# cp2k/dbcsr

Hardware: AMD Instinct MI355X
Metric: block-sparse multiply GFLOP/s (fp64) (higher is better)
Workload: dtype f64; 1 GPU; config2_32768_23x23_fill10_fp64; M=32768, c_nblks=2030625, nproducts=29207882, k_passes=1, parallelism=1 GPU

## Files before the change

### dbcsr_amd/csrc/mm_engine.hip

```cpp
#include <hip/hip_runtime.h>

#include <cstdio>
#include <cstdlib>
#include <cstring>
#include <algorithm>
#include <new>
#include <vector>

#include "../../include/dbcsr_amd_mm.h"
#include "common.h"
#include "smm_core.h"
#include "mm_types.h"
#include "mm_jit.h"

#include "mm_workspace.h"
#include "mm_symbolic.h"
#include "mm_numeric_f64.h"
#include "mm_numeric_f64_big.h"
#include "mm_numeric_f64_small.h"
#include "mm_mid.h"
#include "mm_numeric_f32.h"
#include "mm_aux.h"
#ifdef DBCSR_AMD_EXPERIMENTS
#include "mm_lab_api.h"
#include "mm_group.h"
#include "mm_group64.h"
#include "mm_dma.h"
#include "mm_tile_index.h"
#include "mm_band_index.h"
#endif
namespace dbcsr_amd {

#include "mm_engine_state.h"
#include "mm_engine_env.h"
#include "mm_engine_launch.h"
#include "mm_engine_plan.h"
#ifdef DBCSR_AMD_EXPERIMENTS
#include "mm_engine_lab.h"
#endif


static int build_product_lists(Engine* E, bool reuse, const dbcsr_amd_bcsr* a, const dbcsr_amd_bcsr* b, const dbcsr_amd_bcsr* c_in, dbcsr_amd_bcsr* c_out,
                               hipStream_t st) {
  const int nbr = E->facts.nbr, W = E->W, nbc = b->nblkcols, nJ = (nbc + 63) / 64;
  const int64_t nblk = E->facts.c_nblks;
  const uint32_t* cin_bm = E->have_cin ? E->cin_bm.p : nullptr;
  const int* cin_pre = E->have_cin ? E->cin_pre.p : nullptr;
  if (reuse) {
    ACC_CHECK(hipMemcpyAsync(c_out->col_i, E->plan_c_col_i.p, sizeof(int32_t) * (size_t)nblk, hipMemcpyDeviceToDevice, st));
    ACC_CHECK(hipMemcpyAsync(c_out->blk_p, E->plan_c_blk_p.p, sizeof(int64_t) * (size_t)nblk, hipMemcpyDeviceToDevice, st));
  } else if (E->rows_kernels) {
    if (E->tmp_i32.ensure((size_t)nblk + 1)) return -1;
    ACC_CHECK(hipMemsetAsync(E->tmp_i32.p, 0, sizeof(int) * (size_t)nblk, st));
    hipLaunchKernelGGL(fill_products_rows, grid_for((int64_t)nbr * 64), dim3(256), 0, st, a->row_p, a->col_i, a->blk_p, a->col_blk_size, b->row_p,
                       b->col_i, b->blk_p, E->c_bm.p, E->c_pre.p, c_out->row_p, E->prod_start.p, nbr, W, E->tmp_i32.p, E->entries.p, E->filter);
    hipLaunchKernelGGL(finish_descs_grid, grid_for((int64_t)nbr * nJ * 64), dim3(256), 0, st, c_in->row_p, c_in->blk_p, c_out->row_blk_size,
                       c_out->col_blk_size, cin_bm, cin_pre, E->c_bm.p, E->c_pre.p, c_out->row_p, E->c_blk_p_ws.p, E->prod_start.p,
                       E->prod_cnt.p, nbr, W, nJ, c_out->col_i, c_out->blk_p, E->descs.p);
  } else if (E->grid_kernels) {
    hipLaunchKernelGGL(fill_products_grid, grid_for((int64_t)nbr * nJ * 64), dim3(256), 0, st, a->row_p, a->col_i, a->blk_p, b->row_p,
                       b->blk_p, c_in->row_p, c_in->blk_p, a->row_blk_size, a->col_blk_size, b->col_blk_size, E->b_bm.p, E->b_pre.p,
                       cin_bm, cin_pre, E->c_bm.p, E->c_pre.p, c_out->row_p, E->prod_start.p, E->c_blk_p_ws.p, nbr, nbc, W, nJ, c_out->col_i,
                       c_out->blk_p, E->descs.p, E->entries.p, E->filter);
  } else {
    hipLaunchKernelGGL(fill_products, grid_for((int64_t)nbr * W), dim3(256), 0, st, a->row_p, a->col_i, a->blk_p, b->row_p, b->blk_p,
                       c_in->row_p, c_in->blk_p, a->row_blk_size, a->col_blk_size, b->col_blk_size, E->b_bm.p, E->b_pre.p,
                       cin_bm, cin_pre, E->c_bm.p, E->c_pre.p, c_out->row_p, E->prod_start.p, E->c_blk_p_ws.p, nbr, W, c_out->col_i, c_out->blk_p,
                       E->descs.p, E->entries.p);
  }
  return 0;
}

template <typename T>
static NumericArgs<T> numeric_args(Engine* E, hipStream_t st, const dbcsr_amd_bcsr* a, const dbcsr_amd_bcsr* b, const dbcsr_amd_bcsr* c_in,
                                   const dbcsr_amd_bcsr* c_out, double alpha, double beta, const Work* work, double* norms, bool reuse) {
  return NumericArgs<T>{st, E->descs.p, E->facts.c_nblks, E->entries.p, static_cast<const T*>(a->data), static_cast<const T*>(b->data),
                        static_cast<T*>(c_out->data), static_cast<const T*>(c_in->data), (T)alpha, (T)beta, E->facts.skip_empty, E->order.p, work, norms,
                        a, b, c_out, reuse};
}

static int launch_classes_f64(Engine* E, const NumericArgs<double>& p, const NumericChoice& c) {
  const SizeFacts& F = E->facts;
  int njit = 0, ngen = 0, nmid = 0, jit_mask = 0, nlaunch = 0;
  const int nside = E->lab.class_streams > 1 ? E->lab.class_streams - 1 : 0;
  if (nside) {
    if (!E->fork_ev) ACC_CHECK(hipEventCreateWithFlags(&E->fork_ev, hipEventDisableTiming));
    ACC_CHECK(hipEventRecord(E->fork_ev, p.st));
    for (int i = 0; i < nside; ++i) {
      if (!E->side_stream[i]) {
        ACC_CHECK(hipStreamCreateWithFlags(&E->side_stream[i], hipStreamNonBlocking));
        ACC_CHECK(hipEventCreateWithFlags(&E->join_ev[i], hipEventDisableTiming));
      }
      ACC_CHECK(hipStreamWaitEvent(E->side_stream[i], E->fork_ev, 0));
    }
  }
  for (int k = 0; k < kNumClasses; ++k) {
    if (E->cls_len[k] == 0) continue;
    NumericArgs<double> q = p.segment(E->cls_off[k]);
    const int slot = nlaunch++ % (nside + 1);
    if (slot) q.st = E->side_stream[slot - 1];
    const unsigned npos = (unsigned)(8 * E->cls_len[k]);
    const int cm = k < 9 ? F.cls_m[k / 3] : 0, cn = k < 9 ? F.cls_n[k % 3] : 0;
    ClassKernel ck;
    if (k < 9 && c.mid_class_mode && mid_f64_serves(cm, cn, c.mid_class_mode)) {
      if (!launch_mid_f64(q, (cm + 3) / 4, (cn + 3) / 4, false, npos, (std::max(cm, cn) + 3) / 4)) return -1;
      ++nmid;
      jit_mask |= 1 << k;
    } else if (k < 9 && cm > 0 && cn > 0 && jit_class_kernel(cm, cn, F.cls_k[0], F.cls_k[1], F.cls_k[2], E->lab.class_g, &ck) == 0) {
      long nblk_l = (long)q.nblk;
      void* args[] = {&q.descs, &nblk_l, &q.entries, &q.a, &q.b, &q.c_out, &q.c_in, &q.alpha, &q.beta, &q.skip_empty, &q.order, &q.work, &q.norms};
      const unsigned cw = E->lab.class_g == 1 ? (unsigned)c.ww : 4u;
      ACC_CHECK(hipModuleLaunchKernel(ck.fn, npos / cw / (unsigned)E->lab.class_g, 1, 1, 64 * cw, 1, 1, (unsigned)(cw * ck.wave_lds), q.st, args, nullptr));
      ++njit;
      jit_mask |= 1 << k;
    } else {
      launch_lds_f64(q, c, (unsigned)(8 * E->cls_len[k] / 4) * 4u / (unsigned)c.ww);
      ++ngen;
    }
  }
  for (int i = 0; i < nside; ++i) {
    ACC_CHECK(hipEventRecord(E->join_ev[i], E->side_stream[i]));
    ACC_CHECK(hipStreamWaitEvent(p.st, E->join_ev[i], 0));
  }
  if (p.norms) {
    ClassSet cs;
    for (int r = 0; r < 3; ++r) cs.m[r] = F.cls_m[r], cs.n[r] = F.cls_n[r];
    cs.jit_mask = jit_mask;
    hipLaunchKernelGGL(block_norms_unserved_classes, grid_for(p.nblk * 64), dim3(256), 0, p.st, p.descs, p.nblk, p.c_out, cs, p.norms);
  }
  char slab[24] = "";
  if (nmid > 0) snprintf(slab, sizeof slab, "%d slab + ", nmid);
  snprintf(E->last_kernel, sizeof E->last_kernel, "%s%d jit + %s%d generic launches; m {%d,%d,%d} n {%d,%d,%d} k {%d,%d,%d}]", c.name, njit, slab, ngen,
           F.cls_m[0], F.cls_m[1], F.cls_m[2], F.cls_n[0], F.cls_n[1], F.cls_n[2], F.cls_k[0], F.cls_k[1], F.cls_k[2]);
  return 0;
}

static int launch_f64(Engine* E, const NumericChoice& c, const NumericArgs<double>& p, const LabSwitches& lab) {
  const SizeFacts& F = E->facts;
  const int64_t npos = 8 * F.order_len;
  snprintf(E->last_kernel, sizeof E->last_kernel, "%s", c.name);
  if (p.norms && c.leaves_norms) E->norms_data = p.c_out, E->norms_nblks = p.nblk;
  switch (c.family) {
    case Family::f64_tiny:
      if (c.grid > 0) launch_tiny_f64(p, c, F.max_k <= 4);
      return 0;
    case Family::f64_small8:
      if (c.grid > 0) launch_small_f64(p, c, npos);
      return 0;
    case Family::f64_mid:
      return launch_mid_f64(p, c.mid_rb, c.mid_cb, F.min_m != F.max_m || F.min_n != F.max_n, c.grid, (std::max(F.max_m, F.max_n) + 3) / 4) ? 0 : -1;
    case Family::f64_classes: return launch_classes_f64(E, p, c);
    case Family::f64_hot: return launch_hot_f64(p, c, F.hot_m, F.hot_n, F.hot_k, c.flags, c.variant) ? 0 : -1;
    case Family::f64_pipe: launch_pipe_f64(p, c, npos); return 0;
    case Family::f64_lds: launch_lds_f64(p, c, c.grid); return 0;
    case Family::f64_big: return launch_big_f64(p, c, big_tiles(F.max_m), big_tiles(F.max_n)) ? 0 : -1;
    case Family::f64_generic:
      hipLaunchKernelGGL(mm_numeric_f64, dim3(c.grid), dim3(256), 0, p.st, p.descs, p.nblk, p.entries, p.a, p.b, p.c_out, p.c_in, p.alpha, p.beta, c.flags);
      return 0;
#ifdef DBCSR_AMD_EXPERIMENTS
    case Family::f64_group: case Family::f64_tile: case Family::f64_band: case Family::f64_dma: case Family::f64_persistent: return launch_lab_f64(E, c, p, lab);
#endif
    default: return -1;
  }
}

static int launch_f32(Engine* E, const NumericChoice& c, const NumericArgs<float>& p) {
  const SizeFacts& F = E->facts;
  snprintf(E->last_kernel, sizeof E->last_kernel, "%s", c.name);
  switch (c.family) {
    case Family::f32_classes:
      for (int k = 0; k < kNumClasses; ++k)
        if (E->cls_len[k] != 0) launch_lds_f32(p.segment(E->cls_off[k]), c, (unsigned)(8 * E->cls_len[k] / c.ww));
      return 0;
    case Family::f32_direct: return launch_hot_f32_direct(p, c, F.hot_m, F.hot_n, F.hot_k, c.flags, c.slim) ? 0 : -1;
    case Family::f32_hot: return launch_hot_f32(p, c, F.hot_m, F.hot_n, F.hot_k) ? 0 : -1;
    case Family::f32_lds: launch_lds_f32(p, c, c.grid); return 0;
    case Family::f32_generic:
      hipLaunchKernelGGL(mm_numeric_f32, dim3(c.grid), dim3(256), 0, p.st, p.descs, p.nblk, p.entries, p.a, p.b, p.c_out, p.c_in, p.alpha, p.beta, c.flags);
      return 0;
#ifdef DBCSR_AMD_EXPERIMENTS
    case Family::f32_group: {
      const int rc = run_group_f32(E, p, c.group_R);
      if (rc == 0 && F.other_sizes()) launch_hot_f32_direct(p, c, F.hot_m, F.hot_n, F.hot_k, c.flags | 2, false);
      if (rc != 1) return rc;
      LabSwitches lab = E->lab;
      lab.f32_group = 0;
      return launch_f32(E, choose_numeric(F, E->sw, lab), p);
    }
#endif
    default: return -1;
  }
}

}

using namespace dbcsr_amd;

extern "C" {

int dbcsr_amd_mm_create(void** handle) {
  if (!handle) return -1;
  Engine* E = new (std::nothrow) Engine();
  if (!E) return -1;
  hipError_t e = hipHostMalloc(reinterpret_cast<void**>(&E->host_scalars), 16 * sizeof(int64_t), hipHostMallocDefault);
  if (e != hipSuccess) {
    delete E;
    return check(e, "hipHostMalloc", __FILE__, __LINE__);
  }
  if (hipHostMalloc(reinterpret_cast<void**>(&E->cls_host_hist), 3 * 33 * sizeof(int), hipHostMallocDefault) != hipSuccess ||
      hipHostMalloc(reinterpret_cast<void**>(&E->cls_host_lens), (2 * kNumClasses + 1) * sizeof(int64_t), hipHostMallocDefault) != hipSuccess)
    return -1;
  if (hipHostMalloc(reinterpret_cast<void**>(&E->plan_host_flag), sizeof(int), hipHostMallocDefault) != hipSuccess) return -1;
  engine_read_env(E);
  for (int i = 0; i < 3; ++i) {
    e = hipEventCreate(&E->ev[i]);
    if (e != hipSuccess) return check(e, "hipEventCreate", __FILE__, __LINE__);
  }
  *handle = E;
  return 0;
}

int dbcsr_amd_mm_timing(void* handle, float* ms_fill, float* ms_numeric) {
  Engine* E = static_cast<Engine*>(handle);
  if (!E || !E->timed) return -1;
  ACC_CHECK(hipEventSynchronize(E->ev[2]));
  float f = 0.f, n = 0.f;
  ACC_CHECK(hipEventElapsedTime(&f, E->ev[0], E->ev[1]));
  ACC_CHECK(hipEventElapsedTime(&n, E->ev[1], E->ev[2]));
  if (ms_fill) *ms_fill = f;
  if (ms_numeric) *ms_numeric = n;
  return 0;
}

int dbcsr_amd_mm_destroy(void* handle) {
  if (!handle) return 0;
  Engine* E = static_cast<Engine*>(handle);
  if (E->host_scalars) (void)hipHostFree(E->host_scalars);
  if (E->plan_host_flag) (void)hipHostFree(E->plan_host_flag);
  if (E->cls_host_hist) (void)hipHostFree(E->cls_host_hist);
  if (E->cls_host_lens) (void)hipHostFree(E->cls_host_lens);
  for (int i = 0; i < 3; ++i)
    if (E->ev[i]) (void)hipEventDestroy(E->ev[i]);
  for (int i = 0; i < 3; ++i) {
    if (E->side_stream[i]) (void)hipStreamDestroy(E->side_stream[i]);
    if (E->join_ev[i]) (void)hipEventDestroy(E->join_ev[i]);
  }
  if (E->fork_ev) (void)hipEventDestroy(E->fork_ev);
  delete E;
  return 0;
}

int dbcsr_amd_mm_symbolic(void* handle, const dbcsr_amd_bcsr* a, const dbcsr_amd_bcsr* b, const dbcsr_amd_bcsr* c_in,
                          int retain_sparsity, int32_t* c_out_row_p, dbcsr_amd_mm_counts* counts, void* stream) {
  return dbcsr_amd_mm_symbolic_filtered(handle, dbcsr_type_real_8, 1.0, 0.0, a, b, c_in, retain_sparsity, c_out_row_p, counts, stream);
}

int dbcsr_amd_mm_symbolic_filtered(void* handle, libsmm_acc_data_t datatype, double alpha, double filter_eps, const dbcsr_amd_bcsr* a,
                                   const dbcsr_amd_bcsr* b, const dbcsr_amd_bcsr* c_in, int retain_sparsity, int32_t* c_out_row_p,
                                   dbcsr_amd_mm_counts* counts, void* stream) {
  Engine* E = static_cast<Engine*>(handle);
  if (!E || !a || !b || !c_in || !c_out_row_p || !counts) return -1;
  E->drop_pending = 0.0;
  const bool filtering = filter_eps > 0.0;
  if (filtering && datatype != dbcsr_type_real_8 && datatype != dbcsr_type_real_4) return -10;
  if (a->nblkcols != b->nblkrows || a->nblkrows != c_in->nblkrows || b->nblkcols != c_in->nblkcols) {
    fprintf(stderr, "dbcsr_amd_mm_symbolic: incompatible block dimensions\n");
    return -2;
  }
  hipStream_t st = stream_of(stream);
  const int nbr = a->nblkrows, nbk = a->nblkcols, nbc = b->nblkcols;
  const int W = (nbc + 31) / 32;
  if (!filtering) {
    const int hit = plan_matches(E, a, b, c_in, retain_sparsity ? 1 : 0, st);
    if (hit < 0) return -1;
    if (hit) {
      long long off = 0;
      const void* ptr[12];
      long long n[12];
      plan_segments(a, b, c_in, ptr, n);
      for (int i = 0; i < 12; ++i) off += n[i];
      ACC_CHECK(hipMemcpyAsync(c_out_row_p, E->plan_words.p + off, sizeof(int32_t) * ((size_t)nbr + 1), hipMemcpyDeviceToDevice, st));
      *counts = E->plan_counts;
      E->norms_data = nullptr;
      E->filter = FilterArgs{nullptr, nullptr, 0.0f};
      E->valid = true;
      E->plan_hit = true;
      ++E->plan_hits;
      return 0;
    }
  }
  plan_invalidate(E);
  E->valid = false;
  E->facts.nbr = nbr;
  E->facts.nbc = nbc;
  E->W = W;
  E->facts.retain = retain_sparsity != 0;
  E->norms_data = nullptr;
  E->have_cin = c_in->nblks > 0;
  if (E->b_bm.ensure((size_t)nbk * W + 1) || E->b_pre.ensure((size_t)nbk * W + 1) || E->c_bm.ensure((size_t)nbr * W + 1) ||
      E->c_pre.ensure((size_t)nbr * W + 1) || E->row_nnz.ensure((size_t)nbr + 1) || E->dev_scalars.ensure(16))
    return -1;
  if (E->have_cin && (E->cin_bm.ensure((size_t)nbr * W + 1) || E->cin_pre.ensure((size_t)nbr * W + 1))) return -1;
  ACC_CHECK(hipMemsetAsync(E->dev_scalars.p, 0, 16 * sizeof(unsigned long long), st));
  {
    static const int init[6] = {0, -0x7fffffff, 0, -0x7fffffff, 0, -0x7fffffff};
    ACC_CHECK(hipMemcpyAsync(E->dev_scalars.p + 4, init, sizeof(init), hipMemcpyHostToDevice, st));
  }
  if (nbr == 0 || nbc == 0) {
    ACC_CHECK(hipMemsetAsync(c_out_row_p, 0, sizeof(int32_t) * ((size_t)nbr + 1), st));
    ACC_CHECK(hipStreamSynchronize(st));
    counts->c_nblks = counts->c_nze = counts->nproducts = counts->flop = 0;
    E->facts.c_nblks = 0;
    E->facts.nproducts = 0;
    E->valid = true;
    return 0;
  }
  ACC_CHECK(hipMemsetAsync(E->b_bm.p, 0, sizeof(uint32_t) * (size_t)nbk * W, st));
  if (nbk > 0) {
    hipLaunchKernelGGL(bitmap_from_index, grid_for((int64_t)nbk * 64), dim3(256), 0, st, b->row_p, b->col_i, nbk, W, E->b_bm.p);
    hipLaunchKernelGGL(row_prefix, grid_for((int64_t)nbk * 64), dim3(256), 0, st, E->b_bm.p, nbk, W, E->b_pre.p, (int*)nullptr);
  }
  if (E->have_cin) {
    ACC_CHECK(hipMemsetAsync(E->cin_bm.p, 0, sizeof(uint32_t) * (size_t)nbr * W, st));
    hipLaunchKernelGGL(bitmap_from_index, grid_for((int64_t)nbr * 64), dim3(256), 0, st, c_in->row_p, c_in->col_i, nbr, W,
                       E->cin_bm.p);
    hipLaunchKernelGGL(row_prefix, grid_for((int64_t)nbr * 64), dim3(256), 0, st, E->cin_bm.p, nbr, W, E->cin_pre.p, (int*)nullptr);
  }
  E->filter = FilterArgs{nullptr, nullptr, 0.0f};
  if (filtering) {
    if (E->a_norms.ensure((size_t)a->nblks + 1) || E->b_norms.ensure((size_t)b->nblks + 1)) return -1;
    const int sa = row_split(nbr, a->nblks), sb = row_split(nbk, b->nblks);
    if (datatype == dbcsr_type_real_8) {
      hipLaunchKernelGGL((bcsr_block_norms<double>), grid_for((int64_t)nbr * sa * 64), dim3(256), 0, st, a->row_p, a->col_i, a->blk_p,
                         static_cast<const double*>(a->data), a->row_blk_size, a->col_blk_size, nbr, sa, 1.0, E->a_norms.p, (double*)nullptr);
      hipLaunchKernelGGL((bcsr_block_norms<double>), grid_for((int64_t)nbk * sb * 64), dim3(256), 0, st, b->row_p, b->col_i, b->blk_p,
                         static_cast<const double*>(b->data), b->row_blk_size, b->col_blk_size, nbk, sb, alpha, E->b_norms.p, (double*)nullptr);
    } else {
      hipLaunchKernelGGL((bcsr_block_norms<float>), grid_for((int64_t)nbr * sa * 64), dim3(256), 0, st, a->row_p, a->col_i, a->blk_p,
                         static_cast<const float*>(a->data), a->row_blk_size, a->col_blk_size, nbr, sa, 1.0, E->a_norms.p, (double*)nullptr);
      hipLaunchKernelGGL((bcsr_block_norms<float>), grid_for((int64_t)nbk * sb * 64), dim3(256), 0, st, b->row_p, b->col_i, b->blk_p,
                         static_cast<const float*>(b->data), b->row_blk_size, b->col_blk_size, nbk, sb, alpha, E->b_norms.p, (double*)nullptr);
    }
    E->filter = FilterArgs{E->a_norms.p, E->b_norms.p, (float)filter_eps};
  }
  const double prod_est = (double)a->nblks * ((double)b->nblks / (double)std::max(nbk, 1));
  const bool sparse_guess = E->force_symbolic == 3 || (E->force_symbolic == 0 && nbr >= 2048 && prod_est < 0.6 * (double)nbr * (double)nbc);
  if (filtering && sparse_guess && !retain_sparsity) {
    if (E->have_cin)
      ACC_CHECK(hipMemcpyAsync(E->c_bm.p, E->cin_bm.p, sizeof(uint32_t) * (size_t)nbr * W, hipMemcpyDeviceToDevice, st));
    else
      ACC_CHECK(hipMemsetAsync(E->c_bm.p, 0, sizeof(uint32_t) * (size_t)nbr * W, st));
    hipLaunchKernelGGL(c_bitmap_rows_filtered, grid_for((int64_t)nbr * 64), dim3(256), 0, st, a->row_p, a->col_i, b->row_p, b->col_i, nbr, W,
                       E->facts.canonical_c, E->filter, E->c_bm.p);
  } else if (filtering)
    hipLaunchKernelGGL(c_bitmap_filtered, grid_for((int64_t)nbr * ((nbc + 63) / 64) * 64), dim3(256), 0, st, a->row_p, a->col_i, b->row_p,
                       E->b_bm.p, E->b_pre.p, E->have_cin ? E->cin_bm.p : (const uint32_t*)nullptr, nbr, nbc, W, (nbc + 63) / 64,
                       retain_sparsity ? 1 : 0, E->facts.canonical_c, E->filter, E->c_bm.p);
  else
    hipLaunchKernelGGL(c_bitmap, grid_for((int64_t)nbr * W), dim3(256), 0, st, a->row_p, a->col_i, E->b_bm.p,
                       E->have_cin ? E->cin_bm.p : (const uint32_t*)nullptr, nbr, W, retain_sparsity ? 1 : 0, E->facts.canonical_c, E->c_bm.p);
  hipLaunchKernelGGL(row_prefix, grid_for((int64_t)nbr * 64), dim3(256), 0, st, E->c_bm.p, nbr, W, E->c_pre.p, E->row_nnz.p);
  int64_t* dsc = reinterpret_cast<int64_t*>(E->dev_scalars.p);
  if (exclusive_scan<int32_t>(E, E->row_nnz.p, nbr, c_out_row_p, dsc + 0, true, st)) return -1;
  if (E->sw.use_classes > 0 && E->cls_hist.ensure(3 * 33)) return -1;
  hipLaunchKernelGGL(block_size_stats, dim3(3), dim3(256), 0, st, a->row_blk_size, nbr, a->col_blk_size, nbk, b->col_blk_size, nbc,
                     reinterpret_cast<int*>(E->dev_scalars.p + 4), reinterpret_cast<int*>(E->dev_scalars.p + 8), reinterpret_cast<int*>(E->dev_scalars.p + 11),
                     E->sw.use_classes > 0 ? E->cls_hist.p : (int*)nullptr);
  if (E->sw.use_classes > 0) ACC_CHECK(hipMemcpyAsync(E->cls_host_hist, E->cls_hist.p, 3 * 33 * sizeof(int), hipMemcpyDeviceToHost, st));
  ACC_CHECK(hipMemcpyAsync(E->host_scalars, dsc, 13 * sizeof(int64_t), hipMemcpyDeviceToHost, st));
  ACC_CHECK(hipStreamSynchronize(st));
  const int64_t c_nblks = E->host_scalars[0];
  {
    const int* mx = reinterpret_cast<const int*>(E->host_scalars + 4);
    E->facts.max_m = mx[0]; E->facts.min_m = -mx[1];
    E->facts.max_k = mx[2]; E->facts.min_k = -mx[3];
    E->facts.max_n = mx[4]; E->facts.min_n = -mx[5];
    if (E->facts.max_k > 0xffff || E->facts.max_m > 0x7fff || E->facts.max_n > 0x7fff) {
      fprintf(stderr, "dbcsr_amd_mm_symbolic: block sizes above 32767 (m, n) / 65535 (k) are not supported (packed 16-bit extents)\n");
      return -1;
    }
    const int* md = reinterpret_cast<const int*>(E->host_scalars + 8);
    const bool dominant = 10ll * md[1] >= 9ll * nbr && 10ll * md[3] >= 9ll * nbk && 10ll * md[5] >= 9ll * nbc;
    E->facts.hot_m = dominant ? md[0] : 0;
    E->facts.hot_k = dominant ? md[2] : 0;
    E->facts.hot_n = dominant ? md[4] : 0;
    E->facts.hot_cnt_m = md[1], E->facts.hot_cnt_k = md[3], E->facts.hot_cnt_n = md[5];
    const int* um = reinterpret_cast<const int*>(E->host_scalars + 11);
    E->facts.units_m = um[0], E->facts.units_cnt_m = um[1], E->facts.units_n = um[2], E->facts.units_cnt_n = um[3];
  }
  E->facts.c_nblks = c_nblks;
  choose_classes(&E->facts, E->sw, E->cls_host_hist);
  double mean_k = E->facts.max_k, mean_n = E->facts.max_n;
  if (E->sw.use_classes > 0 && E->facts.max_k <= 32 && E->facts.max_n <= 32 && E->facts.min_k >= 1 && E->facts.min_n >= 1) {
    double sk = 0, ck = 0, sn = 0, cn = 0;
    for (int sz = 1; sz <= 32; ++sz) {
      sn += (double)sz * E->cls_host_hist[33 + sz];
      cn += E->cls_host_hist[33 + sz];
      sk += (double)sz * E->cls_host_hist[66 + sz];
      ck += E->cls_host_hist[66 + sz];
    }
    if (ck > 0 && cn > 0) mean_k = sk / ck, mean_n = sn / cn;
  }
  const int64_t b_bytes_est = (int64_t)((double)b->nblks * mean_k * mean_n * (double)sizeof(double));
  int NP = (int)std::min<int64_t>((b_bytes_est + E->panel_bytes - 1) / E->panel_bytes, (int64_t)W);
  if (NP < 1) NP = 1;
  const int PW = (W + NP - 1) / NP;
  NP = (W + PW - 1) / PW;
  const int R = (nbr + 7) / 8;
  int RG = E->lab.row_group > 0 ? E->lab.row_group : 1;
  RG = std::max(1, std::min(RG, R));
  const int NG = (R + RG - 1) / RG;
  const int nkeys = (E->facts.cls_mode ? kNumClasses : 1) * 8 * NP * (E->facts.cls_mode ? R : NG);
  if (E->order_cnt.ensure((size_t)nkeys + 1) || E->order_base.ensure((size_t)nkeys + 1)) return -1;
  if (E->facts.cls_mode) {
    if (E->cls_row.ensure((size_t)nbr + 1) || E->cls_col.ensure((size_t)nbc + 1) || E->cls_col_bm.ensure((size_t)4 * W + 1) ||
        E->cls_lens.ensure(2 * kNumClasses + 1) || E->cls_vpos.ensure((size_t)nbr + 1) || E->cls_vrow.ensure((size_t)nbr + 1))
      return -1;
    hipLaunchKernelGGL(class_ids, grid_for(nbr), dim3(256), 0, st, a->row_blk_size, nbr, E->facts.cls_m[0], E->facts.cls_m[1], E->facts.cls_m[2], E->cls_row.p);
    hipLaunchKernelGGL(class_ids, grid_for(nbc), dim3(256), 0, st, b->col_blk_size, nbc, E->facts.cls_n[0], E->facts.cls_n[1], E->facts.cls_n[2], E->cls_col.p);
    hipLaunchKernelGGL(class_col_bitmaps, grid_for(W), dim3(256), 0, st, E->cls_col.p, nbc, W, E->cls_col_bm.p);
    hipLaunchKernelGGL(class_row_deal, dim3(1), dim3(256), 0, st, E->cls_row.p, nbr, E->cls_vpos.p, E->cls_vrow.p);
    hipLaunchKernelGGL(order_count_cls, grid_for(nkeys), dim3(256), 0, st, E->c_bm.p, E->cls_row.p, E->cls_col_bm.p, E->cls_vrow.p, nbr, W, PW, NP, R,
                       E->order_cnt.p);
    if (exclusive_scan<int64_t>(E, E->order_cnt.p, nkeys, E->order_base.p, nullptr, false, st)) return -1;
    hipLaunchKernelGGL(order_len_cls, dim3(1), dim3(1), 0, st, E->order_base.p, c_nblks, NP, R, E->cls_lens.p);
    ACC_CHECK(hipMemcpyAsync(E->cls_host_lens, E->cls_lens.p, (2 * kNumClasses + 1) * sizeof(int64_t), hipMemcpyDeviceToHost, st));
  } else {
  hipLaunchKernelGGL(order_count, grid_for(nkeys), dim3(256), 0, st, E->c_pre.p, E->row_nnz.p, nbr, W, PW, NP, NG, RG, E->order_cnt.p);
  if (exclusive_scan<int64_t>(E, E->order_cnt.p, nkeys, E->order_base.p, nullptr, false, st)) return -1;
  hipLaunchKernelGGL(order_len, dim3(1), dim3(1), 0, st, E->order_base.p, c_nblks, NP, NG, dsc + 7);
  }
  if (E->prod_cnt.ensure((size_t)c_nblks + 1) || E->blk_nze.ensure((size_t)c_nblks + 1) || E->prod_start.ensure((size_t)c_nblks + 1) ||
      E->c_blk_p_ws.ensure((size_t)c_nblks + 1))
    return -1;
  const int nJ = (nbc + 63) / 64;
  E->grid_kernels = filtering || (((int64_t)nbr * nJ * 64 <= 256 * std::max<int64_t>(c_nblks, 1)) && !E->force_word_kernels);
  E->rows_kernels = E->force_symbolic == 3 || (E->force_symbolic == 0 && nbr >= 2048 && 10 * c_nblks < 6 * (int64_t)nbr * nbc);
  if (E->rows_kernels) {
    E->grid_kernels = false;
    ACC_CHECK(hipMemsetAsync(E->prod_cnt.p, 0, sizeof(int) * (size_t)c_nblks, st));
    hipLaunchKernelGGL(block_sizes_rows, grid_for((int64_t)nbr * W), dim3(256), 0, st, E->c_bm.p, E->c_pre.p, c_out_row_p, a->row_blk_size,
                       b->col_blk_size, nbr, W, E->blk_nze.p);
    hipLaunchKernelGGL(count_products_rows, grid_for((int64_t)nbr * 64), dim3(256), 0, st, a->row_p, a->col_i, a->row_blk_size, a->col_blk_size,
                       b->col_blk_size, b->row_p, b->col_i, E->c_bm.p, E->c_pre.p, c_out_row_p, nbr, W, E->prod_cnt.p, E->dev_scalars.p + 3,
                       E->filter);
  } else if (E->grid_kernels)
    hipLaunchKernelGGL(count_products_grid, grid_for((int64_t)nbr * nJ * 64), dim3(256), 0, st, a->row_p, a->col_i, a->row_blk_size,
                       a->col_blk_size, b->col_blk_size, E->b_bm.p, E->c_bm.p, E->c_pre.p, c_out_row_p, nbr, nbc, W, nJ,
                       E->prod_cnt.p, E->blk_nze.p, E->dev_scalars.p + 3, b->row_p, E->b_pre.p, E->filter);
  else
    hipLaunchKernelGGL(count_products, grid_for((int64_t)nbr * W), dim3(256), 0, st, a->row_p, a->col_i, a->row_blk_size,
                       a->col_blk_size, b->col_blk_size, E->b_bm.p, E->c_bm.p, E->c_pre.p, c_out_row_p, nbr, W, E->prod_cnt.p,
                       E->blk_nze.p, E->dev_scalars.p + 3);
  if (exclusive_scan<int64_t>(E, E->prod_cnt.p, c_nblks, E->prod_start.p, dsc + 2, false, st)) return -1;
  if (exclusive_scan<int64_t>(E, E->blk_nze.p, c_nblks, E->c_blk_p_ws.p, dsc + 1, false, st)) return -1;
  ACC_CHECK(hipMemcpyAsync(E->host_scalars, dsc, 8 * sizeof(int64_t), hipMemcpyDeviceToHost, st));
  ACC_CHECK(hipStreamSynchronize(st));
  E->facts.order_len = E->host_scalars[7];
  if (E->facts.cls_mode) {
    for (int c = 0; c < kNumClasses; ++c) {
      E->cls_len[c] = E->cls_host_lens[c];
      E->cls_off[c] = E->cls_host_lens[kNumClasses + c];
    }
    const int64_t total = E->cls_host_lens[2 * kNumClasses];
    E->facts.order_len = total / 8;
    if (E->order.ensure((size_t)total + 64)) return -1;
    if (total > 0) {
      ACC_CHECK(hipMemsetAsync(E->order.p, 0xff, sizeof(int) * ((size_t)total + 64), st));
      hipLaunchKernelGGL(order_fill_cls, grid_for((int64_t)nbr * W), dim3(256), 0, st, E->c_bm.p, E->c_pre.p, c_out_row_p, E->cls_row.p,
                         E->cls_col_bm.p, E->order_base.p, E->cls_lens.p, E->cls_vpos.p, nbr, W, PW, NP, R, E->order.p);
    }
  } else {
  if (E->order.ensure((size_t)(8 * E->facts.order_len) + 64)) return -1;
  if (E->facts.order_len > 0) {
    ACC_CHECK(hipMemsetAsync(E->order.p, 0xff, sizeof(int) * ((size_t)(8 * E->facts.order_len) + 64), st));
    hipLaunchKernelGGL(order_fill, grid_for((int64_t)nbr * W), dim3(256), 0, st, E->c_bm.p, E->c_pre.p, E->row_nnz.p, c_out_row_p,
                       E->order_base.p, nbr, W, PW, NP, NG, RG, E->facts.order_len, E->order.p);
  }
  }
  counts->c_nblks = E->host_scalars[0];
  counts->c_nze = E->host_scalars[1];
  counts->nproducts = E->host_scalars[2];
  counts->flop = E->host_scalars[3];
  E->facts.c_nblks = counts->c_nblks;
  E->facts.nproducts = counts->nproducts;
  E->valid = true;
  ++E->plan_misses;
  if (!filtering) {
    if (plan_save(E, a, b, c_in, retain_sparsity ? 1 : 0, c_out_row_p, *counts, st)) return -1;
  } else {
    plan_invalidate(E);
  }
  return check(hipGetLastError(), "dbcsr_amd_mm_symbolic", __FILE__, __LINE__);
}

int dbcsr_amd_mm_numeric(void* handle, libsmm_acc_data_t datatype, double alpha, const dbcsr_amd_bcsr* a, const dbcsr_amd_bcsr* b,
                         double beta, const dbcsr_amd_bcsr* c_in, dbcsr_amd_bcsr* c_out, void* stream) {
  Engine* E = static_cast<Engine*>(handle);
  if (!E || !E->valid || !a || !b || !c_in || !c_out) {
    fprintf(stderr, "dbcsr_amd_mm_numeric: no valid symbolic phase for this handle\n");
    return -1;
  }
  if (datatype != dbcsr_type_real_8 && datatype != dbcsr_type_real_4) return -10;
  hipStream_t st = stream_of(stream);
  SizeFacts& F = E->facts;
  const int64_t nblk = F.c_nblks;
  if (nblk == 0) return 0;
  const bool reuse = E->plan_hit && E->plan_numeric;
  if (!reuse) {
    E->work_built = false;
#ifdef DBCSR_AMD_EXPERIMENTS
    E->ls.forget_plan();
#endif
  }
  if (E->entries.ensure((size_t)F.nproducts + 1) || E->descs.ensure((size_t)nblk + 1)) return -1;
  ACC_CHECK(hipEventRecord(E->ev[0], st));
  if (int rc = build_product_lists(E, reuse, a, b, c_in, c_out, st)) return rc;
  F.nbc = b->nblkcols;
  F.fp64 = datatype == dbcsr_type_real_8;
  F.filter_active = E->filter.a_norms != nullptr;
  F.skip_empty = (c_out->data == c_in->data && F.retain && beta == 1.0) ? 1 : 0;
  const NumericChoice ch = choose_numeric(F, E->sw, E->lab);
  const Work* work = nullptr;
  if (ch.work) {
    const int64_t npos = 8 * F.order_len;
    if (!(reuse && E->work_built)) {
      if (E->work.ensure((size_t)npos + 1)) return -1;
      hipLaunchKernelGGL(build_work, grid_for(npos), dim3(256), 0, st, E->order.p, npos, E->descs.p, nblk, E->entries.p, E->work.p);
      E->work_built = true;
    }
    work = E->work.p;
  }
  double* norms = nullptr;
  E->norms_data = nullptr;
  if (ch.norms) {
    if (E->norms64.ensure((size_t)nblk + 1)) return -1;
    norms = E->norms64.p;
  }
  const double drop = norms ? E->drop_pending : 0.0;
  E->drop_pending = 0.0;
  E->unwritten_below = 0.0;
  if (norms) {
    hipLaunchKernelGGL(store_scalar_f64, dim3(1), dim3(1), 0, st, norms + nblk, drop);
    E->unwritten_below = drop;
  }
  ACC_CHECK(hipEventRecord(E->ev[1], st));
  if ((F.fp64 ? launch_f64(E, ch, numeric_args<double>(E, st, a, b, c_in, c_out, alpha, beta, work, norms, reuse), E->lab)
              : launch_f32(E, ch, numeric_args<float>(E, st, a, b, c_in, c_out, alpha, beta, work, norms, reuse))) != 0) {
    fprintf(stderr, "dbcsr_amd_mm_numeric: launching %s failed\n", E->last_kernel);
    return -1;
  }
  ACC_CHECK(hipEventRecord(E->ev[2], st));
  E->timed = true;
  c_out->nblks = nblk;
  if (E->plan_saved && !E->plan_numeric) {
    if (E->plan_c_col_i.ensure((size_t)nblk + 1) || E->plan_c_blk_p.ensure((size_t)nblk + 1)) return -1;
    ACC_CHECK(hipMemcpyAsync(E->plan_c_col_i.p, c_out->col_i, sizeof(int32_t) * (size_t)nblk, hipMemcpyDeviceToDevice, st));
    ACC_CHECK(hipMemcpyAsync(E->plan_c_blk_p.p, c_out->blk_p, sizeof(int64_t) * (size_t)nblk, hipMemcpyDeviceToDevice, st));
    E->plan_numeric = true;
  }
  return check(hipGetLastError(), "dbcsr_amd_mm_numeric", __FILE__, __LINE__);
}

#include "mm_engine_ops.h"

}
```

### dbcsr_amd/csrc/mm_engine_ops.h

```cpp
#ifndef DBCSR_AMD_MM_ENGINE_OPS_H
#define DBCSR_AMD_MM_ENGINE_OPS_H

int dbcsr_amd_mm_init_c(void* handle, libsmm_acc_data_t datatype, double beta, const dbcsr_amd_bcsr* c_in, dbcsr_amd_bcsr* c_out,
                        void* stream) {
  Engine* E = static_cast<Engine*>(handle);
  if (E) E->plan_numeric = false;
  if (!E || !E->valid || !c_in || !c_out) {
    fprintf(stderr, "dbcsr_amd_mm_init_c: no valid symbolic phase for this handle\n");
    return -1;
  }
  if (datatype != dbcsr_type_real_8 && datatype != dbcsr_type_real_4) return -10;
  hipStream_t st = stream_of(stream);
  const int nbr = E->facts.nbr, W = E->W;
  const int64_t nblk = E->facts.c_nblks;
  c_out->nblks = nblk;
  if (nblk == 0) return 0;
  if (E->descs.ensure((size_t)nblk + 1)) return -1;
  hipLaunchKernelGGL(emit_index, grid_for((int64_t)nbr * W), dim3(256), 0, st, c_in->row_p, c_in->blk_p, c_out->row_blk_size,
                     c_out->col_blk_size, E->have_cin ? E->cin_bm.p : (const uint32_t*)nullptr,
                     E->have_cin ? E->cin_pre.p : (const int*)nullptr, E->c_bm.p, E->c_pre.p, c_out->row_p, E->c_blk_p_ws.p, nbr, W,
                     c_out->col_i, c_out->blk_p, E->descs.p);
  if (datatype == dbcsr_type_real_8)
    hipLaunchKernelGGL((init_c_blocks<double>), grid_for(nblk * 64), dim3(256), 0, st, E->descs.p, nblk,
                       static_cast<double*>(c_out->data), static_cast<const double*>(c_in->data), beta);
  else
    hipLaunchKernelGGL((init_c_blocks<float>), grid_for(nblk * 64), dim3(256), 0, st, E->descs.p, nblk,
                       static_cast<float*>(c_out->data), static_cast<const float*>(c_in->data), (float)beta);
  return check(hipGetLastError(), "dbcsr_amd_mm_init_c", __FILE__, __LINE__);
}


static int element_offsets(Engine* E, const int* sizes, int n, DevBuf<int64_t>& off, hipStream_t st) {
  if (off.ensure((size_t)n + 1)) return -1;
  return exclusive_scan<int64_t>(E, sizes, n, off.p, nullptr, false, st);
}

static Window make_window(const dbcsr_amd_bcsr* m, int64_t row_lo, int64_t row_hi, int64_t col_lo, int64_t col_hi) {
  (void)m;
  const int64_t big = 0x7fffffff;
  Window w;
  w.r0 = (int)(row_lo < 0 ? 0 : row_lo);
  w.r1 = (int)(row_hi < 0 || row_hi > big ? big : row_hi);
  w.c0 = (int)(col_lo < 0 ? 0 : col_lo);
  w.c1 = (int)(col_hi < 0 || col_hi > big ? big : col_hi);
  return w;
}

int dbcsr_amd_bcsr_crop_count(void* handle, libsmm_acc_data_t datatype, const dbcsr_amd_bcsr* m, int64_t row_lo, int64_t row_hi,
                              int64_t col_lo, int64_t col_hi, int32_t* new_row_p, int64_t* new_nblks, int64_t* new_nze, void* stream) {
  Engine* E = static_cast<Engine*>(handle);
  if (E) plan_invalidate(E);
  if (!E || !m || !new_row_p || !new_nblks || !new_nze) return -1;
  if (datatype != dbcsr_type_real_8 && datatype != dbcsr_type_real_4) return -10;
  hipStream_t st = stream_of(stream);
  const int nbr = m->nblkrows;
  const int64_t nb = m->nblks;
  E->valid = false;
  E->flt_nblks = nb;
  E->flt_new_nblks = -1;
  E->crop_win = make_window(m, row_lo, row_hi, col_lo, col_hi);
  E->crop_pending = true;
  if (E->keep.ensure((size_t)nb + 1) || E->blk_nze.ensure((size_t)nb + 1) || E->row_nnz.ensure((size_t)nbr + 1) ||
      E->prod_start.ensure((size_t)nb + 1) || E->c_blk_p_ws.ensure((size_t)nb + 1) || E->dev_scalars.ensure(16))
    return -1;
  int64_t* dsc = reinterpret_cast<int64_t*>(E->dev_scalars.p);
  ACC_CHECK(hipMemsetAsync(dsc, 0, 16 * sizeof(int64_t), st));
  if (element_offsets(E, m->row_blk_size, nbr, E->off_a, st)) return -1;
  if (element_offsets(E, m->col_blk_size, m->nblkcols, E->off_b, st)) return -1;
  if (nbr > 0 && nb > 0)
    hipLaunchKernelGGL(crop_flags, grid_for((int64_t)nbr * 64), dim3(256), 0, st, m->row_p, m->col_i, m->row_blk_size, m->col_blk_size,
                       E->off_a.p, E->off_b.p, nbr, E->crop_win, E->keep.p, E->blk_nze.p, E->row_nnz.p);
  else if (nbr > 0)
    ACC_CHECK(hipMemsetAsync(E->row_nnz.p, 0, sizeof(int) * (size_t)nbr, st));
  if (exclusive_scan<int32_t>(E, E->row_nnz.p, nbr, new_row_p, dsc + 0, true, st)) return -1;
  if (exclusive_scan<int64_t>(E, E->keep.p, nb, E->prod_start.p, nullptr, false, st)) return -1;
  if (exclusive_scan<int64_t>(E, E->blk_nze.p, nb, E->c_blk_p_ws.p, dsc + 1, false, st)) return -1;
  ACC_CHECK(hipMemcpyAsync(E->host_scalars, dsc, 2 * sizeof(int64_t), hipMemcpyDeviceToHost, st));
  ACC_CHECK(hipStreamSynchronize(st));
  *new_nblks = E->host_scalars[0];
  *new_nze = E->host_scalars[1];
  return check(hipGetLastError(), "dbcsr_amd_bcsr_crop_count", __FILE__, __LINE__);
}

int dbcsr_amd_bcsr_crop_apply(void* handle, libsmm_acc_data_t datatype, const dbcsr_amd_bcsr* src, dbcsr_amd_bcsr* dst, void* stream) {
  Engine* E = static_cast<Engine*>(handle);
  if (E) plan_invalidate(E);
  if (!E || !src || !dst || !E->crop_pending || E->flt_nblks != src->nblks) return -1;
  E->crop_pending = false;
  hipStream_t st = stream_of(stream);
  const int nbr = src->nblkrows;
  if (nbr == 0 || src->nblks == 0) return 0;
  if (datatype == dbcsr_type_real_8)
    hipLaunchKernelGGL((crop_compact<double>), grid_for((int64_t)nbr * 64), dim3(256), 0, st, src->row_p, src->col_i, src->blk_p,
                       static_cast<const double*>(src->data), src->row_blk_size, src->col_blk_size, E->off_a.p, E->off_b.p, nbr,
                       E->crop_win, E->keep.p, E->prod_start.p, E->c_blk_p_ws.p, dst->col_i, dst->blk_p, static_cast<double*>(dst->data));
  else if (datatype == dbcsr_type_real_4)
    hipLaunchKernelGGL((crop_compact<float>), grid_for((int64_t)nbr * 64), dim3(256), 0, st, src->row_p, src->col_i, src->blk_p,
                       static_cast<const float*>(src->data), src->row_blk_size, src->col_blk_size, E->off_a.p, E->off_b.p, nbr,
                       E->crop_win, E->keep.p, E->prod_start.p, E->c_blk_p_ws.p, dst->col_i, dst->blk_p, static_cast<float*>(dst->data));
  else
    return -10;
  return check(hipGetLastError(), "dbcsr_amd_bcsr_crop_apply", __FILE__, __LINE__);
}

int dbcsr_amd_bcsr_scale_window(void* handle, libsmm_acc_data_t datatype, dbcsr_amd_bcsr* m, double beta, int64_t row_lo, int64_t row_hi,
                                int64_t col_lo, int64_t col_hi, void* stream) {
  Engine* E = static_cast<Engine*>(handle);
  if (!E || !m) return -1;
  hipStream_t st = stream_of(stream);
  const int nbr = m->nblkrows;
  if (nbr == 0 || m->nblks == 0) return 0;
  const Window w = make_window(m, row_lo, row_hi, col_lo, col_hi);
  if (element_offsets(E, m->row_blk_size, nbr, E->off_a, st)) return -1;
  if (element_offsets(E, m->col_blk_size, m->nblkcols, E->off_b, st)) return -1;
  if (datatype == dbcsr_type_real_8)
    hipLaunchKernelGGL((scale_window<double>), grid_for((int64_t)nbr * 64), dim3(256), 0, st, m->row_p, m->col_i, m->blk_p,
                       static_cast<double*>(m->data), m->row_blk_size, m->col_blk_size, E->off_a.p, E->off_b.p, nbr, w, beta);
  else if (datatype == dbcsr_type_real_4)
    hipLaunchKernelGGL((scale_window<float>), grid_for((int64_t)nbr * 64), dim3(256), 0, st, m->row_p, m->col_i, m->blk_p,
                       static_cast<float*>(m->data), m->row_blk_size, m->col_blk_size, E->off_a.p, E->off_b.p, nbr, w, (float)beta);
  else
    return -10;
  return check(hipGetLastError(), "dbcsr_amd_bcsr_scale_window", __FILE__, __LINE__);
}

int dbcsr_amd_bcsr_filter_count(void* handle, libsmm_acc_data_t datatype, const dbcsr_amd_bcsr* m, double eps, int32_t* new_row_p,
                                int64_t* new_nblks, int64_t* new_nze, void* stream) {
  Engine* E = static_cast<Engine*>(handle);
  if (E) plan_invalidate(E);
  if (!E || !m || !new_row_p || !new_nblks || !new_nze) return -1;
  if (datatype != dbcsr_type_real_8 && datatype != dbcsr_type_real_4) return -10;
  hipStream_t st = stream_of(stream);
  const int nbr = m->nblkrows;
  const int64_t nb = m->nblks;
  E->valid = false;
  E->flt_nblks = nb;
  E->flt_new_nblks = -1;
  if (E->norms64.ensure((size_t)nb + 1) || E->keep.ensure((size_t)nb + 1) || E->blk_nze.ensure((size_t)nb + 1) ||
      E->row_nnz.ensure((size_t)nbr + 1) || E->prod_start.ensure((size_t)nb + 1) || E->c_blk_p_ws.ensure((size_t)nb + 1) ||
      E->dev_scalars.ensure(16))
    return -1;
  int64_t* dsc = reinterpret_cast<int64_t*>(E->dev_scalars.p);
  ACC_CHECK(hipMemsetAsync(dsc, 0, 16 * sizeof(int64_t), st));
  const bool have_norms = E->norms_data != nullptr && E->norms_data == m->data && E->norms_nblks == nb && datatype == dbcsr_type_real_8;
  if (have_norms && E->unwritten_below > eps * eps) {
    fprintf(stderr, "dbcsr_amd_bcsr_filter_count: this matrix was multiplied with a final filter of eps^2 = %g announced (dbcsr_amd_mm_expect_filter); "
                    "blocks below that were not written and cannot be kept with eps^2 = %g\n", E->unwritten_below, eps * eps);
    return -3;
  }
  E->norms_data = nullptr;
  E->unwritten_below = 0.0;
  if (nbr > 0 && nb > 0) {
    const int sm = row_split(nbr, nb);
    if (have_norms) {
    } else if (datatype == dbcsr_type_real_8)
      hipLaunchKernelGGL((bcsr_block_norms<double>), grid_for((int64_t)nbr * sm * 64), dim3(256), 0, st, m->row_p, m->col_i, m->blk_p,
                         static_cast<const double*>(m->data), m->row_blk_size, m->col_blk_size, nbr, sm, 1.0, (float*)nullptr, E->norms64.p);
    else
      hipLaunchKernelGGL((bcsr_block_norms<float>), grid_for((int64_t)nbr * sm * 64), dim3(256), 0, st, m->row_p, m->col_i, m->blk_p,
                         static_cast<const float*>(m->data), m->row_blk_size, m->col_blk_size, nbr, sm, 1.0, (float*)nullptr, E->norms64.p);
    hipLaunchKernelGGL(filter_flags, grid_for((int64_t)nbr * 64), dim3(256), 0, st, E->norms64.p, nb, m->row_p, m->col_i, m->row_blk_size,
                       m->col_blk_size, nbr, eps * eps, E->keep.p, E->blk_nze.p, E->row_nnz.p);
  }
  if (exclusive_scan<int32_t>(E, E->row_nnz.p, nbr, new_row_p, dsc + 0, true, st)) return -1;
  if (exclusive_scan<int64_t>(E, E->keep.p, nb, E->prod_start.p, nullptr, false, st)) return -1;
  if (exclusive_scan<int64_t>(E, E->blk_nze.p, nb, E->c_blk_p_ws.p, dsc + 1, false, st)) return -1;
  ACC_CHECK(hipMemcpyAsync(E->host_scalars, dsc, 2 * sizeof(int64_t), hipMemcpyDeviceToHost, st));
  ACC_CHECK(hipStreamSynchronize(st));
  *new_nblks = E->host_scalars[0];
  *new_nze = E->host_scalars[1];
  E->flt_new_nblks = E->host_scalars[0];
  return check(hipGetLastError(), "dbcsr_amd_bcsr_filter_count", __FILE__, __LINE__);
}

int dbcsr_amd_bcsr_filter_apply(void* handle, libsmm_acc_data_t datatype, const dbcsr_amd_bcsr* src, dbcsr_amd_bcsr* dst, void* stream) {
  Engine* E = static_cast<Engine*>(handle);
  if (E) plan_invalidate(E);
  if (!E || !src || !dst || E->flt_nblks != src->nblks) return -1;
  hipStream_t st = stream_of(stream);
  const int nbr = src->nblkrows;
  if (nbr == 0 || src->nblks == 0) return 0;
  const int sc = row_split(nbr, src->nblks);
  if (datatype == dbcsr_type_real_8)
    hipLaunchKernelGGL((filter_compact<double>), grid_for((int64_t)nbr * sc * 64), dim3(256), 0, st, src->row_p, src->col_i, src->blk_p,
                       static_cast<const double*>(src->data), src->row_blk_size, src->col_blk_size, nbr, sc, E->keep.p, E->prod_start.p,
                       E->c_blk_p_ws.p, dst->col_i, dst->blk_p, static_cast<double*>(dst->data));
  else if (datatype == dbcsr_type_real_4)
    hipLaunchKernelGGL((filter_compact<float>), grid_for((int64_t)nbr * sc * 64), dim3(256), 0, st, src->row_p, src->col_i, src->blk_p,
                       static_cast<const float*>(src->data), src->row_blk_size, src->col_blk_size, nbr, sc, E->keep.p, E->prod_start.p,
                       E->c_blk_p_ws.p, dst->col_i, dst->blk_p, static_cast<float*>(dst->data));
  else
    return -10;
  return check(hipGetLastError(), "dbcsr_amd_bcsr_filter_apply", __FILE__, __LINE__);
}

int dbcsr_amd_bcsr_filter_apply_index(void* handle, const dbcsr_amd_bcsr* src, dbcsr_amd_bcsr* dst, void* stream) {
  Engine* E = static_cast<Engine*>(handle);
  if (E) plan_invalidate(E);
  if (!E || !src || !dst || E->flt_new_nblks < 0 || E->flt_nblks != src->nblks || dst->data != src->data) return -1;
  hipStream_t st = stream_of(stream);
  if (src->nblkrows == 0 || src->nblks == 0 || E->flt_new_nblks == 0) return 0;
  if (!dst->col_i || !dst->blk_p) return -1;
  hipLaunchKernelGGL(filter_compact_index, grid_for(src->nblks), dim3(256), 0, st, src->col_i, src->blk_p, (int64_t)src->nblks, E->keep.p,
                     E->prod_start.p, E->flt_new_nblks, dst->col_i, dst->blk_p);
  return check(hipGetLastError(), "dbcsr_amd_bcsr_filter_apply_index", __FILE__, __LINE__);
}

int dbcsr_amd_mm_set_filter_in_place(void* handle, int on) {
  Engine* E = static_cast<Engine*>(handle);
  if (!E) return -1;
  E->filter_in_place = on ? 1 : 0;
  return 0;
}

int dbcsr_amd_bcsr_checksum(void* handle, libsmm_acc_data_t datatype, const dbcsr_amd_bcsr* m, double* out2, void* stream) {
  Engine* E = static_cast<Engine*>(handle);
  if (!E || !m || !out2) return -1;
  hipStream_t st = stream_of(stream);
  const int nbr = m->nblkrows;
  out2[0] = out2[1] = 0.0;
  if (nbr == 0 || m->nblks == 0) return 0;
  if (E->row_sums.ensure((size_t)2 * nbr + 2)) return -1;
  if (element_offsets(E, m->row_blk_size, nbr, E->off_a, st)) return -1;
  if (element_offsets(E, m->col_blk_size, m->nblkcols, E->off_b, st)) return -1;
  if (datatype == dbcsr_type_real_8)
    hipLaunchKernelGGL((checksum_blocks<double>), grid_for((int64_t)nbr * 64), dim3(256), 0, st, m->row_p, m->col_i, m->blk_p,
                       static_cast<const double*>(m->data), m->row_blk_size, m->col_blk_size, E->off_a.p, E->off_b.p, nbr,
                       E->row_sums.p);
  else if (datatype == dbcsr_type_real_4)
    hipLaunchKernelGGL((checksum_blocks<float>), grid_for((int64_t)nbr * 64), dim3(256), 0, st, m->row_p, m->col_i, m->blk_p,
                       static_cast<const float*>(m->data), m->row_blk_size, m->col_blk_size, E->off_a.p, E->off_b.p, nbr,
                       E->row_sums.p);
  else
    return -10;
  hipLaunchKernelGGL(checksum_final, dim3(1), dim3(256), 0, st, E->row_sums.p, nbr, E->row_sums.p + 2 * (size_t)nbr);
  ACC_CHECK(hipMemcpyAsync(E->host_scalars + 4, E->row_sums.p + 2 * (size_t)nbr, 2 * sizeof(double), hipMemcpyDeviceToHost, st));
  ACC_CHECK(hipStreamSynchronize(st));
  memcpy(out2, E->host_scalars + 4, 2 * sizeof(double));
  return 0;
}

int dbcsr_amd_bcsr_fill_random(void* handle, libsmm_acc_data_t datatype, const dbcsr_amd_bcsr* m, int counter, void* stream) {
  return dbcsr_amd_bcsr_fill_random_dist(handle, datatype, m, counter, nullptr, nullptr, m ? m->nblkrows : 0, stream);
}

int dbcsr_amd_bcsr_fill_random_dist(void* handle, libsmm_acc_data_t datatype, const dbcsr_amd_bcsr* m, int counter,
                                    const int32_t* row_gid, const int32_t* col_gid, int32_t nblkrows_global, void* stream) {
  if (!handle || !m) return -1;
  hipStream_t st = stream_of(stream);
  if (m->nblks == 0) return 0;
  if (datatype == dbcsr_type_real_8)
    hipLaunchKernelGGL(fill_random_f64, grid_for((int64_t)m->nblkrows * 64), dim3(256), 0, st, m->row_p, m->col_i, m->blk_p,
                       static_cast<double*>(m->data), m->row_blk_size, m->col_blk_size, m->nblkrows, m->nblkcols, counter, row_gid, col_gid,
                       nblkrows_global);
  else if (datatype == dbcsr_type_real_4)
    hipLaunchKernelGGL(fill_random_f32, grid_for(m->nblks), dim3(256), 0, st, m->row_p, m->col_i, m->blk_p,
                       static_cast<float*>(m->data), m->row_blk_size, m->col_blk_size, m->nblkrows, m->nblkcols, counter, row_gid, col_gid,
                       nblkrows_global);
  else
    return -10;
  return check(hipGetLastError(), "dbcsr_amd_bcsr_fill_random", __FILE__, __LINE__);
}

int dbcsr_amd_bcsr_transpose(void* handle, libsmm_acc_data_t datatype, const dbcsr_amd_bcsr* src, dbcsr_amd_bcsr* dst, void* stream) {
  Engine* E = static_cast<Engine*>(handle);
  if (E) plan_invalidate(E);
  if (!E || !src || !dst) return -1;
  if (datatype != dbcsr_type_real_8 && datatype != dbcsr_type_real_4) return -10;
  hipStream_t st = stream_of(stream);
  const int s_nbr = src->nblkrows, t_nbr = src->nblkcols;
  const int Wt = (s_nbr + 31) / 32;
  E->valid = false;
  if (E->c_bm.ensure((size_t)t_nbr * Wt + 1) || E->c_pre.ensure((size_t)t_nbr * Wt + 1) || E->row_nnz.ensure((size_t)t_nbr + 1) ||
      E->blk_nze.ensure((size_t)src->nblks + 1) || E->c_blk_p_ws.ensure((size_t)src->nblks + 1))
    return -1;
  if (t_nbr == 0) return 0;
  ACC_CHECK(hipMemsetAsync(E->c_bm.p, 0, sizeof(uint32_t) * (size_t)t_nbr * Wt, st));
  if (s_nbr > 0) hipLaunchKernelGGL(transpose_mark, grid_for((int64_t)s_nbr * 64), dim3(256), 0, st, src->row_p, src->col_i, s_nbr, Wt, E->c_bm.p);
  hipLaunchKernelGGL(row_prefix, grid_for((int64_t)t_nbr * 64), dim3(256), 0, st, E->c_bm.p, t_nbr, Wt, E->c_pre.p, E->row_nnz.p);
  if (exclusive_scan<int32_t>(E, E->row_nnz.p, t_nbr, dst->row_p, nullptr, true, st)) return -1;
  if (src->nblks > 0) {
    hipLaunchKernelGGL(transpose_sizes, grid_for((int64_t)t_nbr * Wt), dim3(256), 0, st, E->c_bm.p, E->c_pre.p, dst->row_p,
                       src->row_blk_size, src->col_blk_size, t_nbr, Wt, E->blk_nze.p);
    if (exclusive_scan<int64_t>(E, E->blk_nze.p, src->nblks, E->c_blk_p_ws.p, nullptr, false, st)) return -1;
    if (datatype == dbcsr_type_real_8)
      hipLaunchKernelGGL((transpose_fill<double>), grid_for((int64_t)s_nbr * 64), dim3(256), 0, st, src->row_p, src->col_i, src->blk_p,
                         static_cast<const double*>(src->data), src->row_blk_size, src->col_blk_size, E->c_bm.p, E->c_pre.p, dst->row_p,
                         E->c_blk_p_ws.p, s_nbr, Wt, dst->col_i, dst->blk_p, static_cast<double*>(dst->data));
    else
      hipLaunchKernelGGL((transpose_fill<float>), grid_for((int64_t)s_nbr * 64), dim3(256), 0, st, src->row_p, src->col_i, src->blk_p,
                         static_cast<const float*>(src->data), src->row_blk_size, src->col_blk_size, E->c_bm.p, E->c_pre.p, dst->row_p,
                         E->c_blk_p_ws.p, s_nbr, Wt, dst->col_i, dst->blk_p, static_cast<float*>(dst->data));
  }
  dst->nblks = src->nblks;
  return check(hipGetLastError(), "dbcsr_amd_bcsr_transpose", __FILE__, __LINE__);
}

int dbcsr_amd_bcsr_desymmetrize_count(void* handle, const dbcsr_amd_bcsr* src, int32_t* dst_row_p, int64_t* nblks, int64_t* nze, void* stream) {
  return dbcsr_amd_bcsr_twin_count(handle, src, 0, dst_row_p, nblks, nze, stream);
}

int dbcsr_amd_bcsr_desymmetrize_apply(void* handle, libsmm_acc_data_t datatype, const dbcsr_amd_bcsr* src, int antisymmetric, dbcsr_amd_bcsr* dst,
                                      void* stream) {
  return dbcsr_amd_bcsr_twin_apply(handle, datatype, src, 0, antisymmetric, dst, stream);
}

int dbcsr_amd_mm_set_canonical_product(void* handle, int on) {
  Engine* E = static_cast<Engine*>(handle);
  if (E) plan_invalidate(E);
  if (!E) return -1;
  E->facts.canonical_c = on ? 1 : 0;
  return 0;
}

int dbcsr_amd_bcsr_twin_count(void* handle, const dbcsr_amd_bcsr* src, int mode, int32_t* dst_row_p, int64_t* nblks, int64_t* nze, void* stream) {
  Engine* E = static_cast<Engine*>(handle);
  if (E) plan_invalidate(E);
  if (!E || !src || !dst_row_p || !nblks || !nze || src->nblkrows != src->nblkcols || mode < 0 || mode > 2) return -1;
  hipStream_t st = stream_of(stream);
  const int nbr = src->nblkrows, W = (nbr + 31) / 32;
  E->valid = false;
  *nblks = *nze = 0;
  if (nbr == 0) return 0;
  if (E->c_bm.ensure((size_t)nbr * W + 1) || E->c_pre.ensure((size_t)nbr * W + 1) || E->row_nnz.ensure((size_t)nbr + 1) ||
      E->blk_nze.ensure(2 * (size_t)src->nblks + 1) || E->c_blk_p_ws.ensure(2 * (size_t)src->nblks + 1) || E->dev_scalars.ensure(16))
    return -1;
  int64_t* dsc = reinterpret_cast<int64_t*>(E->dev_scalars.p);
  ACC_CHECK(hipMemsetAsync(E->c_bm.p, 0, sizeof(uint32_t) * (size_t)nbr * W, st));
  hipLaunchKernelGGL(desym_mark, grid_for((int64_t)nbr * 64), dim3(256), 0, st, src->row_p, src->col_i, nbr, W, mode, E->c_bm.p);
  hipLaunchKernelGGL(row_prefix, grid_for((int64_t)nbr * 64), dim3(256), 0, st, E->c_bm.p, nbr, W, E->c_pre.p, E->row_nnz.p);
  if (exclusive_scan<int32_t>(E, E->row_nnz.p, nbr, dst_row_p, dsc + 0, true, st)) return -1;
  hipLaunchKernelGGL(transpose_sizes, grid_for((int64_t)nbr * W), dim3(256), 0, st, E->c_bm.p, E->c_pre.p, dst_row_p, src->row_blk_size,
                     src->col_blk_size, nbr, W, E->blk_nze.p);
  ACC_CHECK(hipMemcpyAsync(E->host_scalars, dsc, sizeof(int64_t), hipMemcpyDeviceToHost, st));
  ACC_CHECK(hipStreamSynchronize(st));
  *nblks = E->host_scalars[0];
  if (exclusive_scan<int64_t>(E, E->blk_nze.p, *nblks, E->c_blk_p_ws.p, dsc + 1, false, st)) return -1;
  ACC_CHECK(hipMemcpyAsync(E->host_scalars, dsc, 2 * sizeof(int64_t), hipMemcpyDeviceToHost, st));
  ACC_CHECK(hipStreamSynchronize(st));
  *nze = E->host_scalars[1];
  return check(hipGetLastError(), "dbcsr_amd_bcsr_twin_count", __FILE__, __LINE__);
}

int dbcsr_amd_bcsr_twin_apply(void* handle, libsmm_acc_data_t datatype, const dbcsr_amd_bcsr* src, int mode, int antisymmetric, dbcsr_amd_bcsr* dst,
                              void* stream) {
  Engine* E = static_cast<Engine*>(handle);
  if (E) plan_invalidate(E);
  if (!E || !src || !dst || src->nblkrows != src->nblkcols || mode < 0 || mode > 2) return -1;
  if (datatype != dbcsr_type_real_8 && datatype != dbcsr_type_real_4) return -10;
  hipStream_t st = stream_of(stream);
  const int nbr = src->nblkrows, W = (nbr + 31) / 32;
  if (nbr == 0 || src->nblks == 0) return 0;
  if (datatype == dbcsr_type_real_8)
    hipLaunchKernelGGL((desym_fill<double>), grid_for((int64_t)nbr * 64), dim3(256), 0, st, src->row_p, src->col_i, src->blk_p,
                       static_cast<const double*>(src->data), src->row_blk_size, E->c_bm.p, E->c_pre.p, dst->row_p, E->c_blk_p_ws.p, nbr, W,
                       antisymmetric ? -1.0 : 1.0, mode, dst->col_i, dst->blk_p, static_cast<double*>(dst->data));
  else
    hipLaunchKernelGGL((desym_fill<float>), grid_for((int64_t)nbr * 64), dim3(256), 0, st, src->row_p, src->col_i, src->blk_p,
                       static_cast<const float*>(src->data), src->row_blk_size, E->c_bm.p, E->c_pre.p, dst->row_p, E->c_blk_p_ws.p, nbr, W,
                       antisymmetric ? -1.0f : 1.0f, mode, dst->col_i, dst->blk_p, static_cast<float*>(dst->data));
  return check(hipGetLastError(), "dbcsr_amd_bcsr_twin_apply", __FILE__, __LINE__);
}

int dbcsr_amd_mm_stats(void* handle, dbcsr_amd_mnk_stat* out, int max_entries, int* n_entries, void* stream) {
  Engine* E = static_cast<Engine*>(handle);
  if (!E || !n_entries || (max_entries > 0 && !out)) return -1;
  *n_entries = 0;
  if (!E->valid || !E->timed || E->facts.c_nblks == 0) return 0;
  hipStream_t st = stream_of(stream);
  if (E->stat_table.ensure(2 * (size_t)kStatSlots + 2)) return -1;
  unsigned long long* keys = E->stat_table.p;
  unsigned long long* counts = keys + kStatSlots;
  int* overflow = reinterpret_cast<int*>(counts + kStatSlots);
  ACC_CHECK(hipMemsetAsync(keys, 0, sizeof(unsigned long long) * (2 * (size_t)kStatSlots + 2), st));
  hipLaunchKernelGGL(mnk_histogram, grid_for(E->facts.c_nblks), dim3(256), 0, st, E->descs.p, E->facts.c_nblks, E->entries.p, keys, counts, overflow);
  std::vector<unsigned long long> host(2 * (size_t)kStatSlots + 2);
  ACC_CHECK(hipMemcpyAsync(host.data(), keys, sizeof(unsigned long long) * host.size(), hipMemcpyDeviceToHost, st));
  ACC_CHECK(hipStreamSynchronize(st));
  if (*reinterpret_cast<const int*>(&host[2 * (size_t)kStatSlots])) {
    fprintf(stderr, "dbcsr_amd_mm_stats: more than %d distinct (m, n, k) triples\n", kStatSlots);
    return -1;
  }
  std::vector<dbcsr_amd_mnk_stat> all;
  for (int i = 0; i < kStatSlots; ++i)
    if (host[i]) {
      dbcsr_amd_mnk_stat r;
      r.m = (int32_t)(host[i] & 0xffffu);
      r.n = (int32_t)((host[i] >> 16) & 0xffffu);
      r.k = (int32_t)((host[i] >> 32) & 0x7fffffffu);
      r.reserved = 0;
      r.nproducts = (int64_t)host[kStatSlots + i];
      r.flop = 2ll * r.m * r.n * r.k * r.nproducts;
      all.push_back(r);
    }
  std::sort(all.begin(), all.end(), [](const dbcsr_amd_mnk_stat& a, const dbcsr_amd_mnk_stat& b) {
    return a.flop != b.flop ? a.flop > b.flop : (a.m != b.m ? a.m < b.m : (a.n != b.n ? a.n < b.n : a.k < b.k));
  });
  *n_entries = (int)all.size();
  for (int i = 0; i < (int)all.size() && i < max_entries; ++i) out[i] = all[i];
  return 0;
}

const char* dbcsr_amd_mm_kernel_name(libsmm_acc_data_t datatype) {
  return datatype == dbcsr_type_real_4 ? "mm_numeric_f32" : "mm_numeric_f64";
}

const char* dbcsr_amd_mm_last_kernel(void* handle) {
  Engine* E = static_cast<Engine*>(handle);
  return E ? E->last_kernel : "";
}

int dbcsr_amd_mm_expect_filter(void* handle, double eps) {
  Engine* E = static_cast<Engine*>(handle);
  if (!E || !(eps >= 0.0)) return -1;
  E->drop_pending = eps * eps;
  return 0;
}

int dbcsr_amd_mm_trust_plan(void* handle, int on) {
  Engine* E = static_cast<Engine*>(handle);
  if (!E) return -1;
  E->plan_trusted = on != 0;
  return 0;
}

int dbcsr_amd_mm_plan_stats(void* handle, int64_t* reused, int64_t* built) {
  Engine* E = static_cast<Engine*>(handle);
  if (!E) return -1;
  if (reused) *reused = E->plan_hits;
  if (built) *built = E->plan_misses;
  return 0;
}

#ifdef DBCSR_AMD_EXPERIMENTS
int dbcsr_amd_mm_tile_stats(void* handle, int* waves_gave_up, int* list_mismatches) {
  Engine* E = static_cast<Engine*>(handle);
  if (!E) return -1;
  if (strncmp(E->last_kernel, "mm_numeric_f64_tile", 19) != 0 || !E->ls.tile_flags.p) return 1;
  int h[4] = {0, 0, 0, 0};
  ACC_CHECK(hipDeviceSynchronize());
  ACC_CHECK(hipMemcpy(h, E->ls.tile_flags.p, sizeof h, hipMemcpyDeviceToHost));
  if (waves_gave_up) *waves_gave_up = h[0];
  if (list_mismatches) *list_mismatches = h[1];
  if ((E->ls.tile_knobs & 32) && E->ls.tile_times.p) {
    unsigned long long t[8];
    ACC_CHECK(hipMemcpy(t, E->ls.tile_times.p, sizeof t, hipMemcpyDeviceToHost));
    const double w = t[5] ? (double)t[5] : 1.0;
    fprintf(stderr, "dbcsr_amd tile kernel, mean per wave [ms]: total %.3f = window waits %.3f + operand waits %.3f + multiplies %.3f + epilogues %.3f + rest %.3f (%llu waves)\n",
            t[0] / w * 1e-5, t[1] / w * 1e-5, t[2] / w * 1e-5, t[3] / w * 1e-5, t[4] / w * 1e-5, ((double)t[0] - t[1] - t[2] - t[3] - t[4]) / w * 1e-5, t[5]);
  }
  if (getenv("DBCSR_AMD_MM_TILE_VERBOSE"))
    fprintf(stderr, "dbcsr_amd tile kernel: %d waves gave up, %lld reads of the team counters, %lld products waited for the window (of %lld)\n", h[0],
            16ll * h[2], 16ll * h[3], (long long)E->facts.nproducts);
  return 0;
}

int dbcsr_amd_mm_band_stats(void* handle, int* waits_gave_up, int* list_mismatches) {
  Engine* E = static_cast<Engine*>(handle);
  if (!E) return -1;
  if (strncmp(E->last_kernel, "mm_numeric_f64_band", 19) != 0 || !E->ls.band_flags.p) return 1;
  int h[4] = {0, 0, 0, 0};
  ACC_CHECK(hipDeviceSynchronize());
  ACC_CHECK(hipMemcpy(h, E->ls.band_flags.p, sizeof h, hipMemcpyDeviceToHost));
  if (waits_gave_up) *waits_gave_up = h[0];
  if (list_mismatches) *list_mismatches = h[1];
  if ((E->ls.band_knobs & 1) && E->ls.band_times.p) {
    unsigned long long t[16];
    ACC_CHECK(hipMemcpy(t, E->ls.band_times.p, sizeof t, hipMemcpyDeviceToHost));
    const double w = t[5] ? (double)t[5] : 1.0;
    fprintf(stderr,
            "dbcsr_amd band kernel, mean per wave [ms]: total %.3f = window waits %.3f + issue and waits for A %.3f + waits for B %.3f + multiplies %.3f + "
            "epilogues %.3f + rest %.3f (%llu waves; %llu of %lld products waited for their B block, %llu fetched it themselves at the last moment; %llu "
            "fetches waited for the window, %llu reads of the team's counters, %d waves switched the throttle off; %lld list entries, shape %d, ring of %d, window %d)\n",
            t[0] / w * 1e-5, t[8] / w * 1e-5, t[1] / w * 1e-5, t[2] / w * 1e-5, t[3] / w * 1e-5, t[4] / w * 1e-5,
            ((double)t[0] - t[1] - t[2] - t[3] - t[4] - t[8]) / w * 1e-5, t[5], t[7], (long long)E->facts.nproducts, t[6], t[9], t[10], h[3], (long long)E->ls.band_nlist,
            E->ls.band_shape, E->ls.band_depth, E->ls.band_window);
  }
  return 0;
}
#endif

#endif
```

### dbcsr_amd/csrc/mm_engine_state.h

```cpp
#ifndef DBCSR_AMD_MM_ENGINE_STATE_H
#define DBCSR_AMD_MM_ENGINE_STATE_H

struct PlanSegs {
  const int32_t* a[12];
  const int32_t* b[12];
  long long n[12];
  int nseg;
};
__global__ void __launch_bounds__(256) plan_compare(PlanSegs S, int* __restrict__ differs) {
  const long long stride = (long long)gridDim.x * blockDim.x;
  bool bad = false;
  for (int g = 0; g < S.nseg; ++g)
    for (long long i = (long long)blockIdx.x * blockDim.x + threadIdx.x; i < S.n[g]; i += stride) bad |= S.a[g][i] != S.b[g][i];
  if (__ballot(bad) && (threadIdx.x & 63) == 0) atomicOr(differs, 1);
}

#ifdef DBCSR_AMD_EXPERIMENTS
struct LabState {
  int group_R = 0;
  bool group_built = false, b_monotone = false;
  int64_t group_panel_bytes = 0;
  DevBuf<int> groups, group_flag, group_cnt;
  DevBuf<GWork> group_work;
  DevBuf<GEntry> group_entries;
  DevBuf<int64_t> group_start;
  int tile_shape = 0;
  int tile_window = 256, tile_rdv = 0, tile_pub = 1, tile_prefetch = 0, tile_knobs = 0;
  bool tile_built = false, band_built = false;
  DevBuf<uint32_t> a_bm, bt_bm, tile_prog;
  DevBuf<unsigned long long> tile_times;
  DevBuf<int> a_pre, tile_rows, tile_cols, tile_cnt, tile_flags;
  DevBuf<int64_t> tile_start;
  DevBuf<TileDesc> tdescs;
  DevBuf<TileEntry> tentries;
  TileGeom tile_geom = {0, 0, 0, 0, 0, 0, 0, 0, 0, 0, 0, 0};
  int band_shape = 1, band_depth = 20, band_bpol = 0, band_knobs = 0, band_window = 384;
  int64_t band_nlist = 0, band_nrem = 0;
  DevBuf<unsigned> band_prog;
  BandGeom band_geom = {0, 0, 0, 0, 0, 0, 0, 0, 0, 0, 0, 0};
  DevBuf<BandDesc> band_descs_buf;
  DevBuf<BandEntry> band_entries;
  DevBuf<BandRem> band_rem;
  DevBuf<int> band_cnt_list, band_cnt_b, band_cnt_rem, band_sub_cnt, band_flags;
  DevBuf<int64_t> band_list_off, band_seq_off, band_rem_start;
  DevBuf<unsigned long long> band_times;
  unsigned hot_xcd_mask = 0xffu;
  DevBuf<unsigned> hot_counters;

  void forget_plan() { tile_built = band_built = group_built = false; }
};
#endif

struct Engine {
  DevBuf<uint32_t> b_bm, c_bm, cin_bm;
  DevBuf<int> b_pre, c_pre, cin_pre, row_nnz, prod_cnt, blk_nze, tmp_i32;
  DevBuf<int64_t> prod_start, c_blk_p_ws, partial, off_a, off_b;
  DevBuf<Entry> entries;
  DevBuf<Desc> descs;
  DevBuf<double> row_sums, norms64;
  DevBuf<float> a_norms, b_norms;
  DevBuf<int> keep;
  DevBuf<int> order, order_cnt;
  DevBuf<int64_t> order_base;
  DevBuf<Work> work;
  DevBuf<unsigned long long> dev_scalars, stat_table;
  int64_t* host_scalars = nullptr;
  DevBuf<int> cls_hist;
  DevBuf<unsigned char> cls_row, cls_col;
  DevBuf<int> cls_vpos, cls_vrow;
  DevBuf<uint32_t> cls_col_bm;
  DevBuf<int64_t> cls_lens;
  int* cls_host_hist = nullptr;
  int64_t* cls_host_lens = nullptr;
  hipEvent_t ev[3] = {nullptr, nullptr, nullptr};
  hipStream_t side_stream[3] = {nullptr, nullptr, nullptr};
  hipEvent_t fork_ev = nullptr, join_ev[3] = {nullptr, nullptr, nullptr};

  SizeFacts facts;
  int W = 0;
  bool have_cin = false, valid = false;
  bool rows_kernels = false;
  bool grid_kernels = false;
  int64_t cls_len[kNumClasses] = {0}, cls_off[kNumClasses] = {0};
  FilterArgs filter = {nullptr, nullptr, 0.0f};
  double drop_pending = 0.0;
  bool work_built = false;

  const void* norms_data = nullptr;
  int64_t norms_nblks = 0;
  double unwritten_below = 0.0;
  char last_kernel[96] = "";
  bool timed = false;
  int64_t flt_nblks = 0;
  int64_t flt_new_nblks = -1;
  int filter_in_place = 0;
  Window crop_win = {0, 0, 0, 0};
  bool crop_pending = false;
  KPassMemo kpass_memo;

  Switches sw;
  LabSwitches lab;
  int use_plan = 1;
  int force_symbolic = 0;
  bool force_word_kernels = false;
  int64_t panel_bytes = 256ll << 20;

  bool plan_saved = false, plan_hit = false, plan_numeric = false;
  int plan_dims[3] = {0, 0, 0}, plan_retain = 0, plan_canonical = 0, plan_datatype = 0;
  int64_t plan_nblks[3] = {0, 0, 0};
  bool plan_trusted = false;
  const void* plan_ptrs[12] = {nullptr};
  uint64_t plan_stamps[3] = {0, 0, 0};
  DevBuf<int32_t> plan_words, plan_c_col_i;
  DevBuf<int64_t> plan_c_blk_p;
  DevBuf<int> plan_flag;
  int* plan_host_flag = nullptr;
  dbcsr_amd_mm_counts plan_counts = {0, 0, 0, 0};
  long long plan_hits = 0, plan_misses = 0;

#ifdef DBCSR_AMD_EXPERIMENTS
  LabState ls;
#endif
};

KPassMemo* engine_kpass_memo(void* handle) { return handle ? &static_cast<Engine*>(handle)->kpass_memo : nullptr; }
int engine_filter_in_place(void* handle) { return handle ? static_cast<Engine*>(handle)->filter_in_place : 0; }

static inline int row_split(int64_t nbr, int64_t nblks) {
  if (nbr <= 0) return 1;
  const int64_t per_row = nblks / nbr;
  int64_t S = (65536 + nbr - 1) / nbr;
  if (S > per_row) S = per_row;
  return (int)std::max<int64_t>(1, std::min<int64_t>(S, 64));
}

template <typename TO>
static int exclusive_scan(Engine* E, const int* in, int64_t n, TO* out, int64_t* total_dev, bool write_total_at_n, hipStream_t st) {
  const int nb = (int)((n + kScanChunk - 1) / kScanChunk);
  if (E->partial.ensure((size_t)(nb > 0 ? nb : 1))) return -1;
  if (n <= 0) {
    if (total_dev) ACC_CHECK(hipMemsetAsync(total_dev, 0, sizeof(int64_t), st));
    if (write_total_at_n) ACC_CHECK(hipMemsetAsync(out, 0, sizeof(TO), st));
    return 0;
  }
  hipLaunchKernelGGL(scan_reduce, dim3(nb), dim3(kScanThreads), 0, st, in, n, E->partial.p);
  hipLaunchKernelGGL(scan_partials, dim3(1), dim3(kScanThreads), 0, st, E->partial.p, nb, total_dev);
  hipLaunchKernelGGL((scan_apply<TO>), dim3(nb), dim3(kScanThreads), 0, st, in, n, E->partial.p, out, write_total_at_n ? 1 : 0);
  return check(hipGetLastError(), "exclusive_scan", __FILE__, __LINE__);
}

static inline dim3 grid_for(int64_t nthreads) { return dim3((unsigned)((nthreads + 255) / 256)); }

#endif
```

### dbcsr_amd/csrc/mm_symbolic.h

```cpp
#ifndef DBCSR_AMD_MM_SYMBOLIC_H
#define DBCSR_AMD_MM_SYMBOLIC_H
#include "mm_epilogue.h"

namespace dbcsr_amd {


__global__ void __launch_bounds__(256) bitmap_from_index(const int* __restrict__ row_p, const int* __restrict__ col_i, int nbr, int W,
                                                         uint32_t* __restrict__ bm) {
  const int lane = threadIdx.x & 63;
  const int row = (blockIdx.x * blockDim.x + threadIdx.x) >> 6;
  if (row >= nbr) return;
  for (int b = row_p[row] + lane; b < row_p[row + 1]; b += 64) {
    const int j = col_i[b];
    atomicOr(&bm[(size_t)row * W + (j >> 5)], 1u << (j & 31));
  }
}

__device__ __forceinline__ uint32_t canonical_bits(int i, int w) {
  const uint32_t even = (i & 1) ? 0xAAAAAAAAu : 0x55555555u;
  const int d = i - 32 * w;
  const uint32_t upper = d <= 0 ? 0xFFFFFFFFu : (d >= 32 ? 0u : ~((1u << d) - 1u));
  return (even & upper) | (~even & ~upper);
}

__global__ void __launch_bounds__(256) c_bitmap(const int* __restrict__ a_row_p, const int* __restrict__ a_col_i,
                                                const uint32_t* __restrict__ b_bm, const uint32_t* __restrict__ cin_bm, int nbr, int W,
                                                int retain, int canonical, uint32_t* __restrict__ c_bm) {
  const int64_t t = (int64_t)blockIdx.x * blockDim.x + threadIdx.x;
  if (t >= (int64_t)nbr * W) return;
  const int i = (int)(t / W), w = (int)(t % W);
  uint32_t v = 0u;
  if (!retain) {
    for (int ab = a_row_p[i]; ab < a_row_p[i + 1]; ++ab) v |= b_bm[(size_t)a_col_i[ab] * W + w];
    if (canonical) v &= canonical_bits(i, w);
  }
  c_bm[t] = v | (cin_bm ? cin_bm[t] : 0u);
}

__global__ void __launch_bounds__(256) row_prefix(const uint32_t* __restrict__ bm, int nbr, int W, int* __restrict__ pre,
                                                  int* __restrict__ row_nnz) {
  const int lane = threadIdx.x & 63;
  const int row = (blockIdx.x * blockDim.x + threadIdx.x) >> 6;
  if (row >= nbr) return;
  int carry = 0;
  for (int base = 0; base < W; base += 64) {
    const int w = base + lane;
    const int c = w < W ? __popc(bm[(size_t)row * W + w]) : 0;
    int inc = c;
#pragma unroll
    for (int off = 1; off < 64; off <<= 1) {
      const int t = __shfl_up(inc, off, 64);
      if (lane >= off) inc += t;
    }
    if (w < W) pre[(size_t)row * W + w] = carry + inc - c;
    carry += __shfl(inc, 63, 64);
  }
  if (lane == 0 && row_nnz) row_nnz[row] = carry;
}

__global__ void __launch_bounds__(256) count_products(const int* __restrict__ a_row_p, const int* __restrict__ a_col_i,
                                                      const int* __restrict__ rs, const int* __restrict__ ks, const int* __restrict__ cs,
                                                      const uint32_t* __restrict__ b_bm, const uint32_t* __restrict__ c_bm,
                                                      const int* __restrict__ c_pre, const int* __restrict__ c_row_p, int nbr, int W,
                                                      int* __restrict__ prod_cnt, int* __restrict__ blk_nze,
                                                      unsigned long long* __restrict__ flop_out) {
  const int64_t t = (int64_t)blockIdx.x * blockDim.x + threadIdx.x;
  unsigned long long flop = 0;
  if (t < (int64_t)nbr * W) {
    const int i = (int)(t / W), w = (int)(t % W);
    uint32_t v = c_bm[t];
    if (v) {
      const int m = rs[i];
      int cb = c_row_p[i] + c_pre[t];
      const int a0 = a_row_p[i], a1 = a_row_p[i + 1];
      while (v) {
        const int bit = __ffs(v) - 1;
        v &= v - 1;
        const int n = cs[32 * w + bit];
        int cnt = 0;
        long long ksum = 0;
        for (int ab = a0; ab < a1; ++ab) {
          const int k = a_col_i[ab];
          if ((b_bm[(size_t)k * W + w] >> bit) & 1u) {
            ++cnt;
            ksum += ks[k];
          }
        }
        prod_cnt[cb] = cnt;
        blk_nze[cb] = m * n;
        flop += 2ull * (unsigned long long)m * n * ksum;
        ++cb;
      }
    }
  }
  __shared__ unsigned long long red[4];
  flop = wave_sum(flop);
  if ((threadIdx.x & 63) == 0) red[threadIdx.x >> 6] = flop;
  __syncthreads();
  if (threadIdx.x == 0) {
    const unsigned long long s = red[0] + red[1] + red[2] + red[3];
    if (s) atomicAdd(flop_out, s);
  }
}

__global__ void __launch_bounds__(256)
fill_products(const int* __restrict__ a_row_p, const int* __restrict__ a_col_i, const int64_t* __restrict__ a_blk_p,
              const int* __restrict__ b_row_p, const int64_t* __restrict__ b_blk_p, const int* __restrict__ cin_row_p,
              const int64_t* __restrict__ cin_blk_p, const int* __restrict__ rs, const int* __restrict__ ks,
              const int* __restrict__ cs, const uint32_t* __restrict__ b_bm, const int* __restrict__ b_pre,
              const uint32_t* __restrict__ cin_bm, const int* __restrict__ cin_pre, const uint32_t* __restrict__ c_bm,
              const int* __restrict__ c_pre, const int* __restrict__ c_row_p, const int64_t* __restrict__ prod_start,
              const int64_t* __restrict__ c_blk_p_ws, int nbr, int W, int* __restrict__ c_col_i, int64_t* __restrict__ c_blk_p,
              Desc* __restrict__ descs, Entry* __restrict__ entries) {
  const int64_t t = (int64_t)blockIdx.x * blockDim.x + threadIdx.x;
  if (t >= (int64_t)nbr * W) return;
  const int i = (int)(t / W), w = (int)(t % W);
  uint32_t v = c_bm[t];
  if (!v) return;
  const int m = rs[i];
  int cb = c_row_p[i] + c_pre[t];
  const int a0 = a_row_p[i], a1 = a_row_p[i + 1];
  const uint32_t cinw = cin_bm ? cin_bm[t] : 0u;
  while (v) {
    const int bit = __ffs(v) - 1;
    v &= v - 1;
    const uint32_t below = (1u << bit) - 1u;
    const int j = 32 * w + bit;
    int64_t p = prod_start[cb];
    int cnt = 0;
    for (int ab = a0; ab < a1; ++ab) {
      const int k = a_col_i[ab];
      const uint32_t bw = b_bm[(size_t)k * W + w];
      if ((bw >> bit) & 1u) {
        const int bidx = b_row_p[k] + b_pre[(size_t)k * W + w] + __popc(bw & below);
        entries[p + cnt] = Entry::make(a_blk_p[ab], b_blk_p[bidx], ks[k]);
        ++cnt;
      }
    }
    Desc d;
    d.c_off = c_blk_p_ws[cb];
    d.cin_off = -1;
    if ((cinw >> bit) & 1u) d.cin_off = cin_blk_p[cin_row_p[i] + cin_pre[t] + __popc(cinw & below)];
    d.prod_start = p;
    d.prod_cnt = cnt;
    d.m = (int16_t)m;
    d.n = (int16_t)cs[j];
    descs[cb] = d;
    c_col_i[cb] = j;
    c_blk_p[cb] = d.c_off;
    ++cb;
  }
}



struct FilterArgs {
  const float* a_norms;
  const float* b_norms;
  float eps;
};

__device__ __forceinline__ float row_filter_eps(const FilterArgs& F, int nblks_in_a_row) {
  const float e = F.eps / (float)(nblks_in_a_row > 1 ? nblks_in_a_row : 1);
  return e * e;
}

template <typename T>
__global__ void __launch_bounds__(256) bcsr_block_norms(const int* __restrict__ row_p, const int* __restrict__ col_i,
                                                        const int64_t* __restrict__ blk_p, const T* __restrict__ data,
                                                        const int* __restrict__ rs, const int* __restrict__ cs, int nbr, int S, double scale,
                                                        float* __restrict__ norms, double* __restrict__ norms64) {
  const int lane = threadIdx.x & 63;
  const int64_t wv = ((int64_t)blockIdx.x * blockDim.x + threadIdx.x) >> 6;
  const int row = (int)(wv / S), sub = (int)(wv % S);
  if (row >= nbr) return;
  const int m = rs[row];
  for (int b = row_p[row] + sub; b < row_p[row + 1]; b += S) {
    const int ne = m * cs[col_i[b]];
    const T* d = data + blk_p[b];
    double s = 0.0;
    for (int e = lane; e < ne; e += 64) {
      const double x = scale * (double)d[e];
      s += x * x;
    }
    s = wave_sum(s);
    if (lane == 0) {
      if (norms) norms[b] = (float)s;
      if (norms64) norms64[b] = s;
    }
  }
}

__global__ void __launch_bounds__(256) c_bitmap_filtered(const int* __restrict__ a_row_p, const int* __restrict__ a_col_i,
                                                         const int* __restrict__ b_row_p, const uint32_t* __restrict__ b_bm,
                                                         const int* __restrict__ b_pre, const uint32_t* __restrict__ cin_bm, int nbr,
                                                         int nbc, int W, int nJ, int retain, int canonical, FilterArgs F,
                                                         uint32_t* __restrict__ c_bm) {
  const int lane = threadIdx.x & 63;
  const int64_t wv = ((int64_t)blockIdx.x * blockDim.x + threadIdx.x) >> 6;
  if (wv >= (int64_t)nbr * nJ) return;
  const int i = (int)(wv / nJ), jb = (int)(wv % nJ);
  const int j = jb * 64 + lane, w = j >> 5, bit = j & 31;
  bool any = false;
  if (!retain && j < nbc && !(canonical && !((canonical_bits(i, w) >> bit) & 1u))) {
    const int a0 = a_row_p[i], a1 = a_row_p[i + 1];
    const float reps = row_filter_eps(F, a1 - a0);
    const uint32_t below = (1u << bit) - 1u;
    for (int ab = a0; ab < a1; ++ab) {
      const int k = a_col_i[ab];
      const uint32_t bw = b_bm[(size_t)k * W + w];
      if ((bw >> bit) & 1u) {
        const int bidx = b_row_p[k] + b_pre[(size_t)k * W + w] + __popc(bw & below);
        if (!(F.a_norms[ab] * F.b_norms[bidx] < reps)) any = true;
      }
    }
  }
  const unsigned long long mask = __ballot(any);
  if (lane == 0) {
    const int w0 = 2 * jb;
    c_bm[(size_t)i * W + w0] = (uint32_t)mask | (cin_bm ? cin_bm[(size_t)i * W + w0] : 0u);
    if (w0 + 1 < W) c_bm[(size_t)i * W + w0 + 1] = (uint32_t)(mask >> 32) | (cin_bm ? cin_bm[(size_t)i * W + w0 + 1] : 0u);
  }
}


__global__ void __launch_bounds__(256) count_products_grid(const int* __restrict__ a_row_p, const int* __restrict__ a_col_i,
                                                           const int* __restrict__ rs, const int* __restrict__ ks,
                                                           const int* __restrict__ cs, const uint32_t* __restrict__ b_bm,
                                                           const uint32_t* __restrict__ c_bm, const int* __restrict__ c_pre,
                                                           const int* __restrict__ c_row_p, int nbr, int nbc, int W, int nJ,
                                                           int* __restrict__ prod_cnt, int* __restrict__ blk_nze,
                                                           unsigned long long* __restrict__ flop_out, const int* __restrict__ b_row_p,
                                                           const int* __restrict__ b_pre, FilterArgs F) {
  const int lane = threadIdx.x & 63;
  const int64_t wv = ((int64_t)blockIdx.x * blockDim.x + threadIdx.x) >> 6;
  unsigned long long flop = 0;
  if (wv < (int64_t)nbr * nJ) {
    const int i = (int)(wv / nJ), jb = (int)(wv % nJ);
    const int j = jb * 64 + lane, w = j >> 5, bit = j & 31;
    const uint32_t cw = w < W ? c_bm[(size_t)i * W + w] : 0u;
    const bool present = (cw >> bit) & 1u;
    if (__ballot(present)) {
      const int a0 = a_row_p[i], a1 = a_row_p[i + 1];
      const float reps = F.a_norms ? row_filter_eps(F, a1 - a0) : 0.0f;
      int cnt = 0;
      long long ksum = 0;
      for (int ab = a0; ab < a1; ++ab) {
        const int k = a_col_i[ab];
        const uint32_t bw = w < W ? b_bm[(size_t)k * W + w] : 0u;
        if ((bw >> bit) & 1u) {
          if (F.a_norms) {
            const int bidx = b_row_p[k] + b_pre[(size_t)k * W + w] + __popc(bw & ((1u << bit) - 1u));
            if (F.a_norms[ab] * F.b_norms[bidx] < reps) continue;
          }
          ++cnt;
          ksum += ks[k];
        }
      }
      if (present) {
        const int cb = c_row_p[i] + c_pre[(size_t)i * W + w] + __popc(cw & ((1u << bit) - 1u));
        const int m = rs[i], n = cs[j];
        prod_cnt[cb] = cnt;
        blk_nze[cb] = m * n;
        flop = 2ull * (unsigned long long)m * n * (unsigned long long)ksum;
      }
    }
  }
  __shared__ unsigned long long red[4];
  flop = wave_sum(flop);
  if ((threadIdx.x & 63) == 0) red[threadIdx.x >> 6] = flop;
  __syncthreads();
  if (threadIdx.x == 0) {
    const unsigned long long t = red[0] + red[1] + red[2] + red[3];
    if (t) atomicAdd(flop_out, t);
  }
}

__global__ void __launch_bounds__(256)
fill_products_grid(const int* __restrict__ a_row_p, const int* __restrict__ a_col_i, const int64_t* __restrict__ a_blk_p,
                   const int* __restrict__ b_row_p, const int64_t* __restrict__ b_blk_p, const int* __restrict__ cin_row_p,
                   const int64_t* __restrict__ cin_blk_p, const int* __restrict__ rs, const int* __restrict__ ks,
                   const int* __restrict__ cs, const uint32_t* __restrict__ b_bm, const int* __restrict__ b_pre,
                   const uint32_t* __restrict__ cin_bm, const int* __restrict__ cin_pre, const uint32_t* __restrict__ c_bm,
                   const int* __restrict__ c_pre, const int* __restrict__ c_row_p, const int64_t* __restrict__ prod_start,
                   const int64_t* __restrict__ c_blk_p_ws, int nbr, int nbc, int W, int nJ, int* __restrict__ c_col_i,
                   int64_t* __restrict__ c_blk_p, Desc* __restrict__ descs, Entry* __restrict__ entries, FilterArgs F) {
  const int lane = threadIdx.x & 63;
  const int64_t wv = ((int64_t)blockIdx.x * blockDim.x + threadIdx.x) >> 6;
  if (wv >= (int64_t)nbr * nJ) return;
  const int i = (int)(wv / nJ), jb = (int)(wv % nJ);
  const int j = jb * 64 + lane, w = j >> 5, bit = j & 31;
  const uint32_t cw = w < W ? c_bm[(size_t)i * W + w] : 0u;
  const bool present = (cw >> bit) & 1u;
  if (!__ballot(present)) return;
  const uint32_t below = (1u << bit) - 1u;
  const int cb = present ? c_row_p[i] + c_pre[(size_t)i * W + w] + __popc(cw & below) : 0;
  const int64_t p0 = present ? prod_start[cb] : 0;
  const int a0 = a_row_p[i], a1 = a_row_p[i + 1];
  const float reps = F.a_norms ? row_filter_eps(F, a1 - a0) : 0.0f;
  int cnt = 0;
  for (int base = a0; base < a1; base += 64) {
    const int top = min(base + 64, a1);
    unsigned long long hits = 0ull;
    for (int ab = base; ab < top; ++ab) {
      const int k = a_col_i[ab];
      const uint32_t bw = w < W ? b_bm[(size_t)k * W + w] : 0u;
      if (present && ((bw >> bit) & 1u)) hits |= 1ull << (ab - base);
    }
    while (hits) {
      const int ab = base + __ffsll((long long)hits) - 1;
      hits &= hits - 1;
      const int k = a_col_i[ab];
      const uint32_t bw = b_bm[(size_t)k * W + w];
      const int bidx = b_row_p[k] + b_pre[(size_t)k * W + w] + __popc(bw & below);
      if (F.a_norms && F.a_norms[ab] * F.b_norms[bidx] < reps) continue;
      entries[p0 + cnt] = Entry::make(a_blk_p[ab], b_blk_p[bidx], ks[k]);
      ++cnt;
    }
  }
  if (present) {
    Desc d;
    d.c_off = c_blk_p_ws[cb];
    d.cin_off = -1;
    if (cin_bm) {
      const uint32_t cinw = cin_bm[(size_t)i * W + w];
      if ((cinw >> bit) & 1u) d.cin_off = cin_blk_p[cin_row_p[i] + cin_pre[(size_t)i * W + w] + __popc(cinw & below)];
    }
    d.prod_start = p0;
    d.prod_cnt = cnt;
    d.m = (int16_t)rs[i];
    d.n = (int16_t)cs[j];
    descs[cb] = d;
    c_col_i[cb] = j;
    c_blk_p[cb] = d.c_off;
  }
}


__global__ void __launch_bounds__(256) c_bitmap_rows_filtered(const int* __restrict__ a_row_p, const int* __restrict__ a_col_i,
                                                              const int* __restrict__ b_row_p, const int* __restrict__ b_col_i, int nbr, int W,
                                                              int canonical, FilterArgs F, uint32_t* __restrict__ c_bm) {
  const int lane = threadIdx.x & 63;
  const int i = (int)(((int64_t)blockIdx.x * blockDim.x + threadIdx.x) >> 6);
  if (i >= nbr) return;
  const float reps = row_filter_eps(F, a_row_p[i + 1] - a_row_p[i]);
  for (int ab = a_row_p[i]; ab < a_row_p[i + 1]; ++ab) {
    const int k = a_col_i[ab];
    for (int bb = b_row_p[k] + lane; bb < b_row_p[k + 1]; bb += 64) {
      if (F.a_norms[ab] * F.b_norms[bb] < reps) continue;
      const int j = b_col_i[bb], w = j >> 5, bit = j & 31;
      if (canonical && !((canonical_bits(i, w) >> bit) & 1u)) continue;
      atomicOr(&c_bm[(size_t)i * W + w], 1u << bit);
    }
  }
}

__global__ void __launch_bounds__(256) count_products_rows(const int* __restrict__ a_row_p, const int* __restrict__ a_col_i,
                                                           const int* __restrict__ rs, const int* __restrict__ ks, const int* __restrict__ cs,
                                                           const int* __restrict__ b_row_p, const int* __restrict__ b_col_i,
                                                           const uint32_t* __restrict__ c_bm, const int* __restrict__ c_pre,
                                                           const int* __restrict__ c_row_p, int nbr, int W, int* __restrict__ prod_cnt,
                                                           unsigned long long* __restrict__ flop_out, FilterArgs F) {
  const int lane = threadIdx.x & 63;
  const int i = (int)(((int64_t)blockIdx.x * blockDim.x + threadIdx.x) >> 6);
  unsigned long long flop = 0;
  if (i < nbr) {
    const unsigned long long m = (unsigned long long)rs[i];
    const float reps = F.a_norms ? row_filter_eps(F, a_row_p[i + 1] - a_row_p[i]) : 0.0f;
    for (int ab = a_row_p[i]; ab < a_row_p[i + 1]; ++ab) {
      const int k = a_col_i[ab];
      const unsigned long long kk = (unsigned long long)ks[k];
      for (int bb = b_row_p[k] + lane; bb < b_row_p[k + 1]; bb += 64) {
        if (F.a_norms && F.a_norms[ab] * F.b_norms[bb] < reps) continue;
        const int j = b_col_i[bb], w = j >> 5, bit = j & 31;
        const uint32_t cw = c_bm[(size_t)i * W + w];
        if (!((cw >> bit) & 1u)) continue;
        const int cb = c_row_p[i] + c_pre[(size_t)i * W + w] + __popc(cw & ((1u << bit) - 1u));
        atomicAdd(&prod_cnt[cb], 1);
        flop += 2ull * m * (unsigned long long)cs[j] * kk;
      }
    }
  }
  __shared__ unsigned long long red[4];
  flop = wave_sum(flop);
  if (lane == 0) red[threadIdx.x >> 6] = flop;
  __syncthreads();
  if (threadIdx.x == 0) {
    const unsigned long long t = red[0] + red[1] + red[2] + red[3];
    if (t) atomicAdd(flop_out, t);
  }
}

__global__ void __launch_bounds__(256) fill_products_rows(const int* __restrict__ a_row_p, const int* __restrict__ a_col_i,
                                                          const int64_t* __restrict__ a_blk_p, const int* __restrict__ ks,
                                                          const int* __restrict__ b_row_p, const int* __restrict__ b_col_i,
                                                          const int64_t* __restrict__ b_blk_p, const uint32_t* __restrict__ c_bm,
                                                          const int* __restrict__ c_pre, const int* __restrict__ c_row_p,
                                                          const int64_t* __restrict__ prod_start, int nbr, int W, int* __restrict__ fill_cnt,
                                                          Entry* __restrict__ entries, FilterArgs F) {
  const int lane = threadIdx.x & 63;
  const int i = (int)(((int64_t)blockIdx.x * blockDim.x + threadIdx.x) >> 6);
  if (i >= nbr) return;
  const float reps = F.a_norms ? row_filter_eps(F, a_row_p[i + 1] - a_row_p[i]) : 0.0f;
  for (int ab = a_row_p[i]; ab < a_row_p[i + 1]; ++ab) {
    const int k = a_col_i[ab];
    const int kk = ks[k];
    const int64_t a_off = a_blk_p[ab];
    for (int bb = b_row_p[k] + lane; bb < b_row_p[k + 1]; bb += 64) {
      if (F.a_norms && F.a_norms[ab] * F.b_norms[bb] < reps) continue;
      const int j = b_col_i[bb], w = j >> 5, bit = j & 31;
      const uint32_t cw = c_bm[(size_t)i * W + w];
      if (!((cw >> bit) & 1u)) continue;
      const int cb = c_row_p[i] + c_pre[(size_t)i * W + w] + __popc(cw & ((1u << bit) - 1u));
      const int slot = atomicAdd(&fill_cnt[cb], 1);
      entries[prod_start[cb] + slot] = Entry::make(a_off, b_blk_p[bb], kk);
    }
  }
}

__global__ void __launch_bounds__(256) block_sizes_rows(const uint32_t* __restrict__ c_bm, const int* __restrict__ c_pre,
                                                        const int* __restrict__ c_row_p, const int* __restrict__ rs, const int* __restrict__ cs,
                                                        int nbr, int W, int* __restrict__ blk_nze) {
  const int64_t t = (int64_t)blockIdx.x * blockDim.x + threadIdx.x;
  if (t >= (int64_t)nbr * W) return;
  const int i = (int)(t / W), w = (int)(t % W);
  uint32_t v = c_bm[t];
  int cb = c_row_p[i] + c_pre[t];
  while (v) {
    const int bit = __ffs(v) - 1;
    v &= v - 1;
    blk_nze[cb++] = rs[i] * cs[32 * w + bit];
  }
}

__global__ void __launch_bounds__(256)
finish_descs_rows(const int* __restrict__ cin_row_p, const int64_t* __restrict__ cin_blk_p, const int* __restrict__ rs,
                  const int* __restrict__ cs, const uint32_t* __restrict__ cin_bm, const int* __restrict__ cin_pre,
                  const uint32_t* __restrict__ c_bm, const int* __restrict__ c_pre, const int* __restrict__ c_row_p,
                  const int64_t* __restrict__ c_blk_p_ws, const int64_t* __restrict__ prod_start, const int* __restrict__ prod_cnt, int nbr,
                  int W, int* __restrict__ c_col_i, int64_t* __restrict__ c_blk_p, Desc* __restrict__ descs) {
  const int64_t t = (int64_t)blockIdx.x * blockDim.x + threadIdx.x;
  if (t >= (int64_t)nbr * W) return;
  const int i = (int)(t / W), w = (int)(t % W);
  uint32_t v = c_bm[t];
  if (!v) return;
  int cb = c_row_p[i] + c_pre[t];
  const uint32_t cinw = cin_bm ? cin_bm[t] : 0u;
  while (v) {
    const int bit = __ffs(v) - 1;
    v &= v - 1;
    const uint32_t below = (1u << bit) - 1u;
    const int j = 32 * w + bit;
    Desc d;
    d.c_off = c_blk_p_ws[cb];
    d.cin_off = -1;
    if ((cinw >> bit) & 1u) d.cin_off = cin_blk_p[cin_row_p[i] + cin_pre[t] + __popc(cinw & below)];
    d.prod_start = prod_start[cb];
    d.prod_cnt = prod_cnt[cb];
    d.m = (int16_t)rs[i];
    d.n = (int16_t)cs[j];
    descs[cb] = d;
    c_col_i[cb] = j;
    c_blk_p[cb] = d.c_off;
    ++cb;
  }
}

__global__ void __launch_bounds__(256)
finish_descs_grid(const int* __restrict__ cin_row_p, const int64_t* __restrict__ cin_blk_p, const int* __restrict__ rs,
                  const int* __restrict__ cs, const uint32_t* __restrict__ cin_bm, const int* __restrict__ cin_pre,
                  const uint32_t* __restrict__ c_bm, const int* __restrict__ c_pre, const int* __restrict__ c_row_p,
                  const int64_t* __restrict__ c_blk_p_ws, const int64_t* __restrict__ prod_start, const int* __restrict__ prod_cnt, int nbr,
                  int W, int nJ, int* __restrict__ c_col_i, int64_t* __restrict__ c_blk_p, Desc* __restrict__ descs) {
  const int lane = threadIdx.x & 63;
  const int64_t wv = ((int64_t)blockIdx.x * blockDim.x + threadIdx.x) >> 6;
  if (wv >= (int64_t)nbr * nJ) return;
  const int i = (int)(wv / nJ), jb = (int)(wv % nJ);
  const int j = jb * 64 + lane, w = j >> 5, bit = j & 31;
  if (w >= W) return;
  const size_t t = (size_t)i * W + w;
  const uint32_t cw = c_bm[t];
  if (!((cw >> bit) & 1u)) return;
  const uint32_t below = (1u << bit) - 1u;
  const int cb = c_row_p[i] + c_pre[t] + __popc(cw & below);
  Desc d;
  d.c_off = c_blk_p_ws[cb];
  d.cin_off = -1;
  if (cin_bm) {
    const uint32_t cinw = cin_bm[t];
    if ((cinw >> bit) & 1u) d.cin_off = cin_blk_p[cin_row_p[i] + cin_pre[t] + __popc(cinw & below)];
  }
  d.prod_start = prod_start[cb];
  d.prod_cnt = prod_cnt[cb];
  d.m = (int16_t)rs[i];
  d.n = (int16_t)cs[j];
  descs[cb] = d;
  c_col_i[cb] = j;
  c_blk_p[cb] = d.c_off;
}

__global__ void __launch_bounds__(256)
emit_index(const int* __restrict__ cin_row_p, const int64_t* __restrict__ cin_blk_p, const int* __restrict__ rs,
           const int* __restrict__ cs, const uint32_t* __restrict__ cin_bm, const int* __restrict__ cin_pre,
           const uint32_t* __restrict__ c_bm, const int* __restrict__ c_pre, const int* __restrict__ c_row_p,
           const int64_t* __restrict__ c_blk_p_ws, int nbr, int W, int* __restrict__ c_col_i, int64_t* __restrict__ c_blk_p,
           Desc* __restrict__ descs) {
  const int64_t t = (int64_t)blockIdx.x * blockDim.x + threadIdx.x;
  if (t >= (int64_t)nbr * W) return;
  const int i = (int)(t / W), w = (int)(t % W);
  uint32_t v = c_bm[t];
  if (!v) return;
  int cb = c_row_p[i] + c_pre[t];
  const uint32_t cinw = cin_bm ? cin_bm[t] : 0u;
  while (v) {
    const int bit = __ffs(v) - 1;
    v &= v - 1;
    const uint32_t below = (1u << bit) - 1u;
    const int j = 32 * w + bit;
    Desc d;
    d.c_off = c_blk_p_ws[cb];
    d.cin_off = -1;
    if ((cinw >> bit) & 1u) d.cin_off = cin_blk_p[cin_row_p[i] + cin_pre[t] + __popc(cinw & below)];
    d.prod_start = 0;
    d.prod_cnt = 0;
    d.m = (int16_t)rs[i];
    d.n = (int16_t)cs[j];
    descs[cb] = d;
    c_col_i[cb] = j;
    c_blk_p[cb] = d.c_off;
    ++cb;
  }
}

template <typename T>
__global__ void __launch_bounds__(256) init_c_blocks(const Desc* __restrict__ descs, int64_t nblk, T* __restrict__ c_out,
                                                     const T* __restrict__ c_in, T beta) {
  const int lane = threadIdx.x & 63;
  const int64_t cb = ((int64_t)blockIdx.x * blockDim.x + threadIdx.x) >> 6;
  if (cb >= nblk) return;
  const Desc d = descs[cb];
  const int ne = (int)d.m * (int)d.n;
  T* C = c_out + d.c_off;
  if (d.cin_off >= 0) {
    const T* Ci = c_in + d.cin_off;
    for (int e = lane; e < ne; e += 64) C[e] = beta * Ci[e];
  } else {
    for (int e = lane; e < ne; e += 64) C[e] = (T)0;
  }
}

__device__ __forceinline__ int panel_rank(const int* __restrict__ c_pre, const int* __restrict__ row_nnz, int i, int W, int w) {
  return w < W ? c_pre[(size_t)i * W + w] : row_nnz[i];
}

__global__ void __launch_bounds__(256) order_count(const int* __restrict__ c_pre, const int* __restrict__ row_nnz, int nbr, int W, int PW,
                                                   int NP, int NG, int RG, int* __restrict__ cnt) {
  const int key = blockIdx.x * blockDim.x + threadIdx.x;
  if (key >= 8 * NP * NG) return;
  const int g = key % NG, p = (key / NG) % NP, x = key / (NG * NP);
  int c = 0;
  for (int t = 0; t < RG; ++t) {
    const int i = 8 * (g * RG + t) + x;
    if (i < nbr) c += panel_rank(c_pre, row_nnz, i, W, (p + 1) * PW) - panel_rank(c_pre, row_nnz, i, W, p * PW);
  }
  cnt[key] = c;
}

__global__ void __launch_bounds__(256) order_fill(const uint32_t* __restrict__ c_bm, const int* __restrict__ c_pre,
                                                  const int* __restrict__ row_nnz, const int* __restrict__ c_row_p,
                                                  const int64_t* __restrict__ base, int nbr, int W, int PW, int NP, int NG, int RG,
                                                  int64_t len, int* __restrict__ order) {
  const int64_t tid = (int64_t)blockIdx.x * blockDim.x + threadIdx.x;
  if (tid >= (int64_t)nbr * W) return;
  const int i = (int)(tid / W), w = (int)(tid % W);
  uint32_t v = c_bm[tid];
  if (!v) return;
  const int x = i & 7, r = i >> 3, g = r / RG, t = r % RG, p = w / PW;
  const int key = (x * NP + p) * NG + g;
  const int64_t dst0 = (int64_t)x * len + (base[key] - base[(size_t)x * NP * NG]);
  const int w0 = p * PW;
  int cb = c_row_p[i] + c_pre[tid];
  while (v) {
    const int bit = __ffs(v) - 1;
    v &= v - 1;
    const uint32_t below = (1u << bit) - 1u;
    int before = 0;
    for (int tt = 0; tt < RG; ++tt) {
      const int ii = 8 * (g * RG + tt) + x;
      if (ii >= nbr) break;
      const uint32_t ww = c_bm[(size_t)ii * W + w];
      before += c_pre[(size_t)ii * W + w] + __popc(ww & below) - panel_rank(c_pre, row_nnz, ii, W, w0);
      if (tt < t) before += (ww >> bit) & 1u;
    }
    order[dst0 + before] = cb;
    ++cb;
  }
}

__global__ void order_len(const int64_t* __restrict__ base, int64_t total, int NP, int NG, int64_t* __restrict__ out) {
  int64_t mx = 0;
  for (int x = 0; x < 8; ++x) {
    const int64_t b0 = base[(size_t)x * NP * NG];
    const int64_t b1 = x < 7 ? base[(size_t)(x + 1) * NP * NG] : total;
    mx = b1 - b0 > mx ? b1 - b0 : mx;
  }
  out[0] = (mx + 3) & ~(int64_t)3;
}


constexpr int kNumClasses = 10;

__global__ void __launch_bounds__(256) class_ids(const int* __restrict__ sizes, int n, int s0, int s1, int s2, unsigned char* __restrict__ cls) {
  const int i = blockIdx.x * blockDim.x + threadIdx.x;
  if (i >= n) return;
  const int s = sizes[i];
  cls[i] = (unsigned char)(s == s0 ? 0 : (s == s1 ? 1 : (s == s2 ? 2 : 3)));
}

__global__ void __launch_bounds__(256) class_col_bitmaps(const unsigned char* __restrict__ ncls, int nbc, int W, uint32_t* __restrict__ bm) {
  const int w = blockIdx.x * blockDim.x + threadIdx.x;
  if (w >= W) return;
  uint32_t m[4] = {0u, 0u, 0u, 0u};
  for (int b = 0; b < 32; ++b) {
    const int j = 32 * w + b;
    if (j < nbc) m[ncls[j]] |= 1u << b;
  }
  for (int q = 0; q < 4; ++q) bm[(size_t)q * W + w] = m[q];
}

__device__ __forceinline__ uint32_t class_mask(int cls, int rc, const uint32_t* __restrict__ ncls_bm, int W, int w) {
  if (cls < 9) return rc == cls / 3 ? ncls_bm[(size_t)(cls % 3) * W + w] : 0u;
  return rc == 3 ? 0xffffffffu : ncls_bm[(size_t)3 * W + w];
}

__global__ void __launch_bounds__(256) class_row_deal(const unsigned char* __restrict__ rowcls, int nbr, int* __restrict__ vpos, int* __restrict__ vrow) {
  __shared__ int cnt[256][4];
  __shared__ int cls_off[4];
  const int t = threadIdx.x, chunk = (nbr + 255) / 256, i0 = t * chunk, i1 = min(nbr, i0 + chunk);
  int c[4] = {0, 0, 0, 0};
  for (int i = i0; i < i1; ++i) ++c[rowcls[i]];
  for (int q = 0; q < 4; ++q) cnt[t][q] = c[q];
  __syncthreads();
  if (t < 4) {
    int run = 0;
    for (int u = 0; u < 256; ++u) {
      const int v = cnt[u][t];
      cnt[u][t] = run;
      run += v;
    }
    cls_off[t] = run;
  }
  __syncthreads();
  if (t == 0) {
    int run = 0;
    for (int q = 0; q < 4; ++q) {
      const int v = cls_off[q];
      cls_off[q] = run;
      run += v;
    }
  }
  __syncthreads();
  int at[4];
  for (int q = 0; q < 4; ++q) at[q] = cls_off[q] + cnt[t][q];
  for (int i = i0; i < i1; ++i) {
    const int j = at[rowcls[i]]++;
    vpos[i] = j;
    vrow[j] = i;
  }
}

__global__ void __launch_bounds__(256) order_count_cls(const uint32_t* __restrict__ c_bm, const unsigned char* __restrict__ rowcls,
                                                       const uint32_t* __restrict__ ncls_bm, const int* __restrict__ vrow, int nbr, int W, int PW, int NP, int R,
                                                       int* __restrict__ cnt) {
  const int key = blockIdx.x * blockDim.x + threadIdx.x;
  if (key >= kNumClasses * 8 * NP * R) return;
  const int g = key % R, p = (key / R) % NP, x = (key / (R * NP)) % 8, cls = key / (R * NP * 8);
  const int j = 8 * g + x;
  int c = 0;
  if (j < nbr) {
    const int i = vrow[j];
    const int rc = rowcls[i];
    const int w1 = min(W, (p + 1) * PW);
    for (int w = p * PW; w < w1; ++w) c += __popc(c_bm[(size_t)i * W + w] & class_mask(cls, rc, ncls_bm, W, w));
  }
  cnt[key] = c;
}

__global__ void order_len_cls(const int64_t* __restrict__ base, int64_t total, int NP, int R, int64_t* __restrict__ lens ) {
  int64_t off = 0;
  for (int cls = 0; cls < kNumClasses; ++cls) {
    int64_t mx = 0;
    for (int x = 0; x < 8; ++x) {
      const size_t k0 = ((size_t)cls * 8 + x) * NP * R, k1 = k0 + (size_t)NP * R;
      const int64_t b1 = (cls == kNumClasses - 1 && x == 7) ? total : base[k1];
      mx = b1 - base[k0] > mx ? b1 - base[k0] : mx;
    }
    const int64_t len = (mx + 31) & ~(int64_t)31;
    lens[cls] = len;
    lens[kNumClasses + cls] = off;
    off += 8 * len;
  }
  lens[2 * kNumClasses] = off;
}

__global__ void __launch_bounds__(256) order_fill_cls(const uint32_t* __restrict__ c_bm, const int* __restrict__ c_pre,
                                                      const int* __restrict__ c_row_p, const unsigned char* __restrict__ rowcls,
                                                      const uint32_t* __restrict__ ncls_bm, const int64_t* __restrict__ base,
                                                      const int64_t* __restrict__ lens, const int* __restrict__ vpos, int nbr, int W, int PW, int NP,
                                                      int R, int* __restrict__ order) {
  const int64_t tid = (int64_t)blockIdx.x * blockDim.x + threadIdx.x;
  if (tid >= (int64_t)nbr * W) return;
  const int i = (int)(tid / W), w = (int)(tid % W);
  uint32_t v = c_bm[tid];
  if (!v) return;
  const int j = vpos[i];
  const int x = j & 7, g = j >> 3, p = w / PW, rc = rowcls[i];
  int before[4] = {0, 0, 0, 0};
  for (int ww = p * PW; ww < w; ++ww) {
    const uint32_t cw = c_bm[(size_t)i * W + ww];
    if (rc == 3)
      before[3] += __popc(cw);
    else
      for (int q = 0; q < 4; ++q) before[q] += __popc(cw & ncls_bm[(size_t)q * W + ww]);
  }
  int cb = c_row_p[i] + c_pre[tid];
  while (v) {
    const int bit = __ffs(v) - 1;
    v &= v - 1;
    int q = 3;
    if (rc != 3)
      for (int qq = 0; qq < 3; ++qq)
        if ((ncls_bm[(size_t)qq * W + w] >> bit) & 1u) q = qq;
    const int cls = (rc < 3 && q < 3) ? rc * 3 + q : 9;
    const size_t key = (((size_t)cls * 8 + x) * NP + p) * R + g;
    const size_t key0 = ((size_t)cls * 8 + x) * NP * R;
    const int64_t pos = lens[kNumClasses + cls] + (int64_t)x * lens[cls] + (base[key] - base[key0]) + before[q];
    order[pos] = cb;
    ++before[q];
    ++cb;
  }
}

}
#endif
```

### dbcsr_amd/csrc/mm_workspace.h

```cpp
#ifndef DBCSR_AMD_MM_WORKSPACE_H
#define DBCSR_AMD_MM_WORKSPACE_H

namespace dbcsr_amd {

static int g_devbuf_poison = -1;

template <typename T>
struct DevBuf {
  T* p = nullptr;
  size_t cap = 0;
  DevBuf() = default;
  DevBuf(const DevBuf&) = delete;
  DevBuf& operator=(const DevBuf&) = delete;
  ~DevBuf() { release(); }
  int ensure(size_t n) {
    if (n <= cap) return 0;
    if (p) (void)hipFree(p);
    p = nullptr;
    cap = 0;
    size_t want = n + n / 8 + 64;
    hipError_t e = hipMalloc(reinterpret_cast<void**>(&p), want * sizeof(T));
    if (e != hipSuccess) return check(e, "hipMalloc(workspace)", __FILE__, __LINE__);
    cap = want;
    if (g_devbuf_poison >= 0) (void)hipMemset(p, g_devbuf_poison, want * sizeof(T));
    return 0;
  }
  void release() {
    if (p) (void)hipFree(p);
    p = nullptr;
    cap = 0;
  }
};


constexpr int kScanThreads = 256;
constexpr int kScanItems = 16;
constexpr int kScanChunk = kScanThreads * kScanItems;

__device__ __forceinline__ int64_t block_exclusive_scan(int64_t v, int64_t* total) {
  __shared__ int64_t wsum[kScanThreads / 64];
  const int lane = threadIdx.x & 63, w = threadIdx.x >> 6;
  int64_t inc = v;
#pragma unroll
  for (int off = 1; off < 64; off <<= 1) {
    const int64_t t = __shfl_up(inc, off, 64);
    if (lane >= off) inc += t;
  }
  if (lane == 63) wsum[w] = inc;
  __syncthreads();
  int64_t woff = 0, tot = 0;
#pragma unroll
  for (int i = 0; i < kScanThreads / 64; ++i) {
    if (i < w) woff += wsum[i];
    tot += wsum[i];
  }
  __syncthreads();
  *total = tot;
  return woff + inc - v;
}

__global__ void __launch_bounds__(kScanThreads) scan_reduce(const int* __restrict__ in, int64_t n, int64_t* __restrict__ partial) {
  const int64_t base = (int64_t)blockIdx.x * kScanChunk;
  int64_t s = 0;
  for (int it = 0; it < kScanItems; ++it) {
    const int64_t i = base + (int64_t)it * kScanThreads + threadIdx.x;
    if (i < n) s += in[i];
  }
  int64_t tot;
  (void)block_exclusive_scan(s, &tot);
  if (threadIdx.x == 0) partial[blockIdx.x] = tot;
}

__global__ void __launch_bounds__(kScanThreads) scan_partials(int64_t* __restrict__ partial, int np, int64_t* __restrict__ total_out) {
  int64_t carry = 0;
  for (int base = 0; base < np; base += kScanThreads) {
    const int i = base + threadIdx.x;
    const int64_t v = i < np ? partial[i] : 0;
    int64_t tot;
    const int64_t ex = block_exclusive_scan(v, &tot);
    if (i < np) partial[i] = carry + ex;
    carry += tot;
  }
  if (threadIdx.x == 0 && total_out) *total_out = carry;
}

template <typename TO>
__global__ void __launch_bounds__(kScanThreads) scan_apply(const int* __restrict__ in, int64_t n, const int64_t* __restrict__ partial,
                                                            TO* __restrict__ out, int write_total_at_n) {
  const int64_t base = (int64_t)blockIdx.x * kScanChunk;
  const int64_t first = base + (int64_t)threadIdx.x * kScanItems;
  int v[kScanItems];
  int64_t s = 0;
#pragma unroll
  for (int it = 0; it < kScanItems; ++it) {
    const int64_t i = first + it;
    v[it] = i < n ? in[i] : 0;
    s += v[it];
  }
  int64_t tot;
  int64_t ex = block_exclusive_scan(s, &tot) + partial[blockIdx.x];
#pragma unroll
  for (int it = 0; it < kScanItems; ++it) {
    const int64_t i = first + it;
    if (i < n) out[i] = (TO)ex;
    ex += v[it];
    if (write_total_at_n && i == n - 1) out[n] = (TO)ex;
  }
}

}
#endif
```

Baseline: 37500 GFLOP/s.

## Count products per bitmap word and fuse counting into C bitmap pass

Replaces per-block product counting and scans in the grid symbolic path with per-bitmap-word counts and offsets. In the unfiltered case the product counts and flops are computed inside the c_bitmap kernel, using precomputed B word sizes. The fill kernel then derives per-block product and C offsets with in-wave prefix sums, and can stage entries in LDS before copying them out coalesced. This cuts the number of symbolic passes and shrinks the scans from c_nblks to nbr*W entries, at the cost of more complex kernels, extra LDS use and heavier c_bitmap work.

After: 37520 GFLOP/s (median of 2 runs). Within noise of the previous version (+0.0%).

```diff
diff --git a/dbcsr_amd/csrc/mm_engine.hip b/dbcsr_amd/csrc/mm_engine.hip
--- a/dbcsr_amd/csrc/mm_engine.hip
+++ b/dbcsr_amd/csrc/mm_engine.hip
@@ -39,6 +39,8 @@
 #include "mm_engine_lab.h"
 #endif
 
+
+static inline int64_t F_nproducts_per_wave(int64_t nproducts, int64_t nwaves) { return nproducts / std::max<int64_t>(nwaves, 1); }
 
 static int build_product_lists(Engine* E, bool reuse, const dbcsr_amd_bcsr* a, const dbcsr_amd_bcsr* b, const dbcsr_amd_bcsr* c_in, dbcsr_amd_bcsr* c_out,
                                hipStream_t st) {
@@ -58,10 +60,14 @@
                        c_out->col_blk_size, cin_bm, cin_pre, E->c_bm.p, E->c_pre.p, c_out->row_p, E->c_blk_p_ws.p, E->prod_start.p,
                        E->prod_cnt.p, nbr, W, nJ, c_out->col_i, c_out->blk_p, E->descs.p);
   } else if (E->grid_kernels) {
-    hipLaunchKernelGGL(fill_products_grid, grid_for((int64_t)nbr * nJ * 64), dim3(256), 0, st, a->row_p, a->col_i, a->blk_p, b->row_p,
-                       b->blk_p, c_in->row_p, c_in->blk_p, a->row_blk_size, a->col_blk_size, b->col_blk_size, E->b_bm.p, E->b_pre.p,
-                       cin_bm, cin_pre, E->c_bm.p, E->c_pre.p, c_out->row_p, E->prod_start.p, E->c_blk_p_ws.p, nbr, nbc, W, nJ, c_out->col_i,
-                       c_out->blk_p, E->descs.p, E->entries.p, E->filter);
+    const int64_t per_wave = F_nproducts_per_wave(E->facts.nproducts, (int64_t)nbr * nJ);
+    const int cap = (per_wave >= 64 && per_wave + per_wave / 8 <= kListStageCap) ? kListStageCap : 0;
+    const int threads = cap ? 64 : 256;
+    const size_t lds = (size_t)(threads / 64) * (64 * sizeof(KRec) + (size_t)cap * sizeof(Entry));
+    hipLaunchKernelGGL(list_products_grid, dim3((unsigned)(((int64_t)nbr * nJ * 64 + threads - 1) / threads)), dim3(threads), lds, st, a->row_p,
+                       a->col_i, a->blk_p, b->row_p, b->blk_p, c_in->row_p, c_in->blk_p, a->row_blk_size, a->col_blk_size, b->col_blk_size,
+                       E->b_bm.p, E->b_pre.p, cin_bm, cin_pre, E->c_bm.p, E->c_pre.p, c_out->row_p, E->word_pstart.p, E->word_cstart.p, nbr, W,
+                       nJ, cap, c_out->col_i, c_out->blk_p, E->descs.p, E->entries.p, E->filter);
   } else {
     hipLaunchKernelGGL(fill_products, grid_for((int64_t)nbr * W), dim3(256), 0, st, a->row_p, a->col_i, a->blk_p, b->row_p, b->blk_p,
                        c_in->row_p, c_in->blk_p, a->row_blk_size, a->col_blk_size, b->col_blk_size, E->b_bm.p, E->b_pre.p,
@@ -344,6 +350,7 @@
     E->filter = FilterArgs{E->a_norms.p, E->b_norms.p, (float)filter_eps};
   }
   const double prod_est = (double)a->nblks * ((double)b->nblks / (double)std::max(nbk, 1));
+  bool word_counted = false;
   const bool sparse_guess = E->force_symbolic == 3 || (E->force_symbolic == 0 && nbr >= 2048 && prod_est < 0.6 * (double)nbr * (double)nbc);
   if (filtering && sparse_guess && !retain_sparsity) {
     if (E->have_cin)
@@ -356,9 +363,18 @@
     hipLaunchKernelGGL(c_bitmap_filtered, grid_for((int64_t)nbr * ((nbc + 63) / 64) * 64), dim3(256), 0, st, a->row_p, a->col_i, b->row_p,
                        E->b_bm.p, E->b_pre.p, E->have_cin ? E->cin_bm.p : (const uint32_t*)nullptr, nbr, nbc, W, (nbc + 63) / 64,
                        retain_sparsity ? 1 : 0, E->facts.canonical_c, E->filter, E->c_bm.p);
-  else
+  else {
+    word_counted = !E->force_word_kernels && !sparse_guess && nbk > 0;
+    if (word_counted) {
+      if (E->b_wsum.ensure((size_t)nbk * W + 1) || E->word_cnt.ensure((size_t)nbr * W + 1)) return -1;
+      hipLaunchKernelGGL((word_sizes<int>), grid_for((int64_t)nbk * W), dim3(256), 0, st, E->b_bm.p, (const int*)nullptr, b->col_blk_size, nbk, W,
+                         E->b_wsum.p);
+    }
     hipLaunchKernelGGL(c_bitmap, grid_for((int64_t)nbr * W), dim3(256), 0, st, a->row_p, a->col_i, E->b_bm.p,
-                       E->have_cin ? E->cin_bm.p : (const uint32_t*)nullptr, nbr, W, retain_sparsity ? 1 : 0, E->facts.canonical_c, E->c_bm.p);
+                       E->have_cin ? E->cin_bm.p : (const uint32_t*)nullptr, nbr, W, retain_sparsity ? 1 : 0, E->facts.canonical_c, E->c_bm.p,
+                       a->row_blk_size, a->col_blk_size, b->col_blk_size, E->b_wsum.p, word_counted ? E->word_cnt.p : (int*)nullptr,
+                       E->dev_scalars.p + 13);
+  }
   hipLaunchKernelGGL(row_prefix, grid_for((int64_t)nbr * 64), dim3(256), 0, st, E->c_bm.p, nbr, W, E->c_pre.p, E->row_nnz.p);
   int64_t* dsc = reinterpret_cast<int64_t*>(E->dev_scalars.p);
   if (exclusive_scan<int32_t>(E, E->row_nnz.p, nbr, c_out_row_p, dsc + 0, true, st)) return -1;
@@ -430,31 +446,44 @@
   if (exclusive_scan<int64_t>(E, E->order_cnt.p, nkeys, E->order_base.p, nullptr, false, st)) return -1;
   hipLaunchKernelGGL(order_len, dim3(1), dim3(1), 0, st, E->order_base.p, c_nblks, NP, NG, dsc + 7);
   }
-  if (E->prod_cnt.ensure((size_t)c_nblks + 1) || E->blk_nze.ensure((size_t)c_nblks + 1) || E->prod_start.ensure((size_t)c_nblks + 1) ||
-      E->c_blk_p_ws.ensure((size_t)c_nblks + 1))
-    return -1;
   const int nJ = (nbc + 63) / 64;
   E->grid_kernels = filtering || (((int64_t)nbr * nJ * 64 <= 256 * std::max<int64_t>(c_nblks, 1)) && !E->force_word_kernels);
   E->rows_kernels = E->force_symbolic == 3 || (E->force_symbolic == 0 && nbr >= 2048 && 10 * c_nblks < 6 * (int64_t)nbr * nbc);
-  if (E->rows_kernels) {
-    E->grid_kernels = false;
-    ACC_CHECK(hipMemsetAsync(E->prod_cnt.p, 0, sizeof(int) * (size_t)c_nblks, st));
-    hipLaunchKernelGGL(block_sizes_rows, grid_for((int64_t)nbr * W), dim3(256), 0, st, E->c_bm.p, E->c_pre.p, c_out_row_p, a->row_blk_size,
-                       b->col_blk_size, nbr, W, E->blk_nze.p);
-    hipLaunchKernelGGL(count_products_rows, grid_for((int64_t)nbr * 64), dim3(256), 0, st, a->row_p, a->col_i, a->row_blk_size, a->col_blk_size,
-                       b->col_blk_size, b->row_p, b->col_i, E->c_bm.p, E->c_pre.p, c_out_row_p, nbr, W, E->prod_cnt.p, E->dev_scalars.p + 3,
-                       E->filter);
-  } else if (E->grid_kernels)
-    hipLaunchKernelGGL(count_products_grid, grid_for((int64_t)nbr * nJ * 64), dim3(256), 0, st, a->row_p, a->col_i, a->row_blk_size,
-                       a->col_blk_size, b->col_blk_size, E->b_bm.p, E->c_bm.p, E->c_pre.p, c_out_row_p, nbr, nbc, W, nJ,
-                       E->prod_cnt.p, E->blk_nze.p, E->dev_scalars.p + 3, b->row_p, E->b_pre.p, E->filter);
-  else
-    hipLaunchKernelGGL(count_products, grid_for((int64_t)nbr * W), dim3(256), 0, st, a->row_p, a->col_i, a->row_blk_size,
-                       a->col_blk_size, b->col_blk_size, E->b_bm.p, E->c_bm.p, E->c_pre.p, c_out_row_p, nbr, W, E->prod_cnt.p,
-                       E->blk_nze.p, E->dev_scalars.p + 3);
-  if (exclusive_scan<int64_t>(E, E->prod_cnt.p, c_nblks, E->prod_start.p, dsc + 2, false, st)) return -1;
-  if (exclusive_scan<int64_t>(E, E->blk_nze.p, c_nblks, E->c_blk_p_ws.p, dsc + 1, false, st)) return -1;
-  ACC_CHECK(hipMemcpyAsync(E->host_scalars, dsc, 8 * sizeof(int64_t), hipMemcpyDeviceToHost, st));
+  if (E->rows_kernels) E->grid_kernels = false;
+  bool flop_from_c_bitmap = false;
+  if (E->grid_kernels) {
+    if (E->word_cnt.ensure((size_t)nbr * W + 1) || E->word_nze.ensure((size_t)nbr * W + 1) || E->word_pstart.ensure((size_t)nbr * W + 1) ||
+        E->word_cstart.ensure((size_t)nbr * W + 1))
+      return -1;
+    if (word_counted)
+      flop_from_c_bitmap = true;
+    else
+      hipLaunchKernelGGL(count_products_words, grid_for((int64_t)nbr * nJ * 64), dim3(256), 0, st, a->row_p, a->col_i, a->blk_p, b->row_p,
+                         a->row_blk_size, a->col_blk_size, b->col_blk_size, E->b_bm.p, E->b_pre.p, E->c_bm.p, nbr, W, nJ, E->word_cnt.p,
+                         E->dev_scalars.p + 3, E->filter);
+    hipLaunchKernelGGL((word_sizes<int64_t>), grid_for((int64_t)nbr * W), dim3(256), 0, st, E->c_bm.p, a->row_blk_size, b->col_blk_size, nbr, W,
+                       E->word_nze.p);
+    if (exclusive_scan<int64_t>(E, E->word_cnt.p, (int64_t)nbr * W, E->word_pstart.p, dsc + 2, false, st)) return -1;
+    if (exclusive_scan<int64_t>(E, E->word_nze.p, (int64_t)nbr * W, E->word_cstart.p, dsc + 1, false, st)) return -1;
+  } else {
+    if (E->prod_cnt.ensure((size_t)c_nblks + 1) || E->blk_nze.ensure((size_t)c_nblks + 1) || E->prod_start.ensure((size_t)c_nblks + 1) ||
+        E->c_blk_p_ws.ensure((size_t)c_nblks + 1))
+      return -1;
+    if (E->rows_kernels) {
+      ACC_CHECK(hipMemsetAsync(E->prod_cnt.p, 0, sizeof(int) * (size_t)c_nblks, st));
+      hipLaunchKernelGGL(block_sizes_rows, grid_for((int64_t)nbr * W), dim3(256), 0, st, E->c_bm.p, E->c_pre.p, c_out_row_p, a->row_blk_size,
+                         b->col_blk_size, nbr, W, E->blk_nze.p);
+      hipLaunchKernelGGL(count_products_rows, grid_for((int64_t)nbr * 64), dim3(256), 0, st, a->row_p, a->col_i, a->row_blk_size, a->col_blk_size,
+                         b->col_blk_size, b->row_p, b->col_i, E->c_bm.p, E->c_pre.p, c_out_row_p, nbr, W, E->prod_cnt.p, E->dev_scalars.p + 3,
+                         E->filter);
+    } else
+      hipLaunchKernelGGL(count_products, grid_for((int64_t)nbr * W), dim3(256), 0, st, a->row_p, a->col_i, a->row_blk_size,
+                         a->col_blk_size, b->col_blk_size, E->b_bm.p, E->c_bm.p, E->c_pre.p, c_out_row_p, nbr, W, E->prod_cnt.p,
+                         E->blk_nze.p, E->dev_scalars.p + 3);
+    if (exclusive_scan<int64_t>(E, E->prod_cnt.p, c_nblks, E->prod_start.p, dsc + 2, false, st)) return -1;
+    if (exclusive_scan<int64_t>(E, E->blk_nze.p, c_nblks, E->c_blk_p_ws.p, dsc + 1, false, st)) return -1;
+  }
+  ACC_CHECK(hipMemcpyAsync(E->host_scalars, dsc, 14 * sizeof(int64_t), hipMemcpyDeviceToHost, st));
   ACC_CHECK(hipStreamSynchronize(st));
   E->facts.order_len = E->host_scalars[7];
   if (E->facts.cls_mode) {
@@ -481,7 +510,7 @@
   counts->c_nblks = E->host_scalars[0];
   counts->c_nze = E->host_scalars[1];
   counts->nproducts = E->host_scalars[2];
-  counts->flop = E->host_scalars[3];
+  counts->flop = E->host_scalars[flop_from_c_bitmap ? 13 : 3];
   E->facts.c_nblks = counts->c_nblks;
   E->facts.nproducts = counts->nproducts;
   E->valid = true;
diff --git a/dbcsr_amd/csrc/mm_engine_ops.h b/dbcsr_amd/csrc/mm_engine_ops.h
--- a/dbcsr_amd/csrc/mm_engine_ops.h
+++ b/dbcsr_amd/csrc/mm_engine_ops.h
@@ -18,8 +18,8 @@
   if (E->descs.ensure((size_t)nblk + 1)) return -1;
   hipLaunchKernelGGL(emit_index, grid_for((int64_t)nbr * W), dim3(256), 0, st, c_in->row_p, c_in->blk_p, c_out->row_blk_size,
                      c_out->col_blk_size, E->have_cin ? E->cin_bm.p : (const uint32_t*)nullptr,
-                     E->have_cin ? E->cin_pre.p : (const int*)nullptr, E->c_bm.p, E->c_pre.p, c_out->row_p, E->c_blk_p_ws.p, nbr, W,
-                     c_out->col_i, c_out->blk_p, E->descs.p);
+                     E->have_cin ? E->cin_pre.p : (const int*)nullptr, E->c_bm.p, E->c_pre.p, c_out->row_p, E->c_blk_p_ws.p,
+                     E->grid_kernels ? E->word_cstart.p : (const int64_t*)nullptr, nbr, W, c_out->col_i, c_out->blk_p, E->descs.p);
   if (datatype == dbcsr_type_real_8)
     hipLaunchKernelGGL((init_c_blocks<double>), grid_for(nblk * 64), dim3(256), 0, st, E->descs.p, nblk,
                        static_cast<double*>(c_out->data), static_cast<const double*>(c_in->data), beta);
diff --git a/dbcsr_amd/csrc/mm_engine_state.h b/dbcsr_amd/csrc/mm_engine_state.h
--- a/dbcsr_amd/csrc/mm_engine_state.h
+++ b/dbcsr_amd/csrc/mm_engine_state.h
@@ -55,6 +55,8 @@
   DevBuf<uint32_t> b_bm, c_bm, cin_bm;
   DevBuf<int> b_pre, c_pre, cin_pre, row_nnz, prod_cnt, blk_nze, tmp_i32;
   DevBuf<int64_t> prod_start, c_blk_p_ws, partial, off_a, off_b;
+  DevBuf<int> b_wsum, word_cnt;
+  DevBuf<int64_t> word_nze, word_pstart, word_cstart;
   DevBuf<Entry> entries;
   DevBuf<Desc> descs;
   DevBuf<double> row_sums, norms64;
@@ -134,8 +136,8 @@
   return (int)std::max<int64_t>(1, std::min<int64_t>(S, 64));
 }
 
-template <typename TO>
-static int exclusive_scan(Engine* E, const int* in, int64_t n, TO* out, int64_t* total_dev, bool write_total_at_n, hipStream_t st) {
+template <typename TO, typename TI>
+static int exclusive_scan(Engine* E, const TI* in, int64_t n, TO* out, int64_t* total_dev, bool write_total_at_n, hipStream_t st) {
   const int nb = (int)((n + kScanChunk - 1) / kScanChunk);
   if (E->partial.ensure((size_t)(nb > 0 ? nb : 1))) return -1;
   if (n <= 0) {
@@ -143,9 +145,9 @@
     if (write_total_at_n) ACC_CHECK(hipMemsetAsync(out, 0, sizeof(TO), st));
     return 0;
   }
-  hipLaunchKernelGGL(scan_reduce, dim3(nb), dim3(kScanThreads), 0, st, in, n, E->partial.p);
+  hipLaunchKernelGGL((scan_reduce<TI>), dim3(nb), dim3(kScanThreads), 0, st, in, n, E->partial.p);
   hipLaunchKernelGGL(scan_partials, dim3(1), dim3(kScanThreads), 0, st, E->partial.p, nb, total_dev);
-  hipLaunchKernelGGL((scan_apply<TO>), dim3(nb), dim3(kScanThreads), 0, st, in, n, E->partial.p, out, write_total_at_n ? 1 : 0);
+  hipLaunchKernelGGL((scan_apply<TO, TI>), dim3(nb), dim3(kScanThreads), 0, st, in, n, E->partial.p, out, write_total_at_n ? 1 : 0);
   return check(hipGetLastError(), "exclusive_scan", __FILE__, __LINE__);
 }
 
diff --git a/dbcsr_amd/csrc/mm_symbolic.h b/dbcsr_amd/csrc/mm_symbolic.h
--- a/dbcsr_amd/csrc/mm_symbolic.h
+++ b/dbcsr_amd/csrc/mm_symbolic.h
@@ -23,18 +23,68 @@
   return (even & upper) | (~even & ~upper);
 }
 
+template <typename TO>
+__global__ void __launch_bounds__(256) word_sizes(const uint32_t* __restrict__ bm, const int* __restrict__ scale, const int* __restrict__ cs, int nrows, int W,
+                                                  TO* __restrict__ out) {
+  const int64_t t = (int64_t)blockIdx.x * blockDim.x + threadIdx.x;
+  if (t >= (int64_t)nrows * W) return;
+  const int w = (int)(t % W);
+  uint32_t v = bm[t];
+  TO s = 0;
+  while (v) {
+    s += cs[32 * w + __ffs(v) - 1];
+    v &= v - 1;
+  }
+  out[t] = scale ? s * (TO)scale[t / W] : s;
+}
+
 __global__ void __launch_bounds__(256) c_bitmap(const int* __restrict__ a_row_p, const int* __restrict__ a_col_i,
                                                 const uint32_t* __restrict__ b_bm, const uint32_t* __restrict__ cin_bm, int nbr, int W,
-                                                int retain, int canonical, uint32_t* __restrict__ c_bm) {
+                                                int retain, int canonical, uint32_t* __restrict__ c_bm, const int* __restrict__ rs,
+                                                const int* __restrict__ ks, const int* __restrict__ cs, const int* __restrict__ b_wsum,
+                                                int* __restrict__ word_cnt, unsigned long long* __restrict__ flop_out) {
   const int64_t t = (int64_t)blockIdx.x * blockDim.x + threadIdx.x;
-  if (t >= (int64_t)nbr * W) return;
-  const int i = (int)(t / W), w = (int)(t % W);
-  uint32_t v = 0u;
-  if (!retain) {
-    for (int ab = a_row_p[i]; ab < a_row_p[i + 1]; ++ab) v |= b_bm[(size_t)a_col_i[ab] * W + w];
+  unsigned long long flop = 0;
+  if (t < (int64_t)nbr * W) {
+    const int i = (int)(t / W), w = (int)(t % W);
+    const uint32_t cin = cin_bm ? cin_bm[t] : 0u;
+    uint32_t v = 0u;
+    if (word_cnt) {
+      const uint32_t adm = retain ? cin : (canonical ? (canonical_bits(i, w) | cin) : 0xFFFFFFFFu);
+      int cnt = 0;
+      unsigned long long kn = 0;
+      for (int ab = a_row_p[i]; ab < a_row_p[i + 1]; ++ab) {
+        const int k = a_col_i[ab];
+        const uint32_t bw = b_bm[(size_t)k * W + w];
+        v |= bw;
+        uint32_t h = bw & adm;
+        if (!h) continue;
+        cnt += __popc(h);
+        int nsum = 0;
+        if (h == bw)
+          nsum = b_wsum[(size_t)k * W + w];
+        else
+          for (; h; h &= h - 1) nsum += cs[32 * w + __ffs(h) - 1];
+        kn += (unsigned long long)ks[k] * (unsigned long long)nsum;
+      }
+      word_cnt[t] = cnt;
+      flop = 2ull * (unsigned long long)rs[i] * kn;
+    } else if (!retain) {
+      for (int ab = a_row_p[i]; ab < a_row_p[i + 1]; ++ab) v |= b_bm[(size_t)a_col_i[ab] * W + w];
+    }
+    if (retain) v = 0u;
     if (canonical) v &= canonical_bits(i, w);
-  }
-  c_bm[t] = v | (cin_bm ? cin_bm[t] : 0u);
+    c_bm[t] = v | cin;
+  }
+  if (!word_cnt) return;
+  __shared__ unsigned long long red[4];
+  flop = wave_sum(flop);
+  if ((threadIdx.x & 63) == 0) red[threadIdx.x >> 6] = flop;
+  __syncthreads();
+  if (threadIdx.x == 0) {
+    const unsigned long long s = red[0] + red[1] + red[2] + red[3];
+    if (s) atomicAdd(flop_out, s);
+  }
 }
 
 __global__ void __launch_bounds__(256) row_prefix(const uint32_t* __restrict__ bm, int nbr, int W, int* __restrict__ pre,
@@ -224,112 +274,223 @@
 }
 
 
-__global__ void __launch_bounds__(256) count_products_grid(const int* __restrict__ a_row_p, const int* __restrict__ a_col_i,
-                                                           const int* __restrict__ rs, const int* __restrict__ ks,
-                                                           const int* __restrict__ cs, const uint32_t* __restrict__ b_bm,
-                                                           const uint32_t* __restrict__ c_bm, const int* __restrict__ c_pre,
-                                                           const int* __restrict__ c_row_p, int nbr, int nbc, int W, int nJ,
-                                                           int* __restrict__ prod_cnt, int* __restrict__ blk_nze,
-                                                           unsigned long long* __restrict__ flop_out, const int* __restrict__ b_row_p,
-                                                           const int* __restrict__ b_pre, FilterArgs F) {
+struct KRec {
+  int64_t a_off;
+  int ks, bb0, bb1;
+  uint32_t bw0, bw1;
+  float a_norm;
+};
+constexpr int kListStageCap = 1024;
+
+__device__ __forceinline__ unsigned long long transpose_bits64(unsigned long long x, int lane) {
+#pragma unroll
+  for (int j = 32; j; j >>= 1) {
+    const unsigned long long m = ~0ull / ((1ull << j) + 1ull);
+    const unsigned long long o = __shfl_xor(x, j, 64);
+    if (lane & j)
+      x ^= ((o >> j) ^ x) & m;
+    else
+      x ^= (((x >> j) ^ o) & m) << j;
+  }
+  return x;
+}
+
+struct GridWalk {
+  int lane, W, w0, a1;
+  bool has1, present;
+  uint32_t below;
+  float reps;
+  KRec* rec;
+};
+
+__device__ __forceinline__ unsigned long long grid_walk_chunk(const GridWalk& g, int base, const int* __restrict__ a_col_i,
+                                                              const int64_t* __restrict__ a_blk_p, const int* __restrict__ ks,
+                                                              const int* __restrict__ b_row_p, const uint32_t* __restrict__ b_bm,
+                                                              const int* __restrict__ b_pre, const FilterArgs& F) {
+  const int ab = base + g.lane;
+  KRec r = {0, 0, 0, 0, 0u, 0u, 0.0f};
+  if (ab < g.a1) {
+    const int k = a_col_i[ab];
+    const size_t t = (size_t)k * g.W + g.w0;
+    r.bw0 = b_bm[t];
+    r.bw1 = g.has1 ? b_bm[t + 1] : 0u;
+    r.bb0 = b_row_p[k] + b_pre[t];
+    r.bb1 = r.bb0 + __popc(r.bw0);
+    r.a_off = a_blk_p[ab];
+    r.ks = ks[k];
+    if (F.a_norms) r.a_norm = F.a_norms[ab];
+  }
+  __builtin_amdgcn_wave_barrier();
+  DBCSR_AMD_LDS_ORDER();
+  g.rec[g.lane] = r;
+  DBCSR_AMD_LDS_ORDER();
+  __builtin_amdgcn_wave_barrier();
+  const unsigned long long col = transpose_bits64((unsigned long long)r.bw0 | ((unsigned long long)r.bw1 << 32), g.lane);
+  return g.present ? col : 0ull;
+}
+
+__device__ __forceinline__ int grid_b_index(const GridWalk& g, const KRec& r) {
+  return g.lane < 32 ? r.bb0 + __popc(r.bw0 & g.below) : r.bb1 + __popc(r.bw1 & g.below);
+}
+
+__device__ __forceinline__ unsigned long long grid_filter_hits(const GridWalk& g, unsigned long long hits, const FilterArgs& F) {
+  unsigned long long keep = 0ull;
+  while (hits) {
+    const int l = __ffsll((long long)hits) - 1;
+    hits &= hits - 1;
+    const KRec r = g.rec[l];
+    if (!(r.a_norm * F.b_norms[grid_b_index(g, r)] < g.reps)) keep |= 1ull << l;
+  }
+  return keep;
+}
+
+__device__ __forceinline__ GridWalk grid_walk_setup(int lane, int i, int jb, int W, const int* __restrict__ a_row_p, const uint32_t* __restrict__ c_bm,
+                                                    const FilterArgs& F, KRec* rec, int* a0, unsigned long long* cmask) {
+  GridWalk g;
+  g.lane = lane, g.W = W, g.w0 = 2 * jb, g.has1 = 2 * jb + 1 < W, g.rec = rec;
+  const uint32_t cw0 = c_bm[(size_t)i * W + g.w0], cw1 = g.has1 ? c_bm[(size_t)i * W + g.w0 + 1] : 0u;
+  *cmask = (unsigned long long)cw0 | ((unsigned long long)cw1 << 32);
+  g.present = (*cmask >> lane) & 1ull;
+  g.below = (1u << (lane & 31)) - 1u;
+  *a0 = a_row_p[i];
+  g.a1 = a_row_p[i + 1];
+  g.reps = F.a_norms ? row_filter_eps(F, g.a1 - *a0) : 0.0f;
+  return g;
+}
+
+__global__ void __launch_bounds__(256) count_products_words(const int* __restrict__ a_row_p, const int* __restrict__ a_col_i,
+                                                            const int64_t* __restrict__ a_blk_p, const int* __restrict__ b_row_p,
+                                                            const int* __restrict__ rs, const int* __restrict__ ks, const int* __restrict__ cs,
+                                                            const uint32_t* __restrict__ b_bm, const int* __restrict__ b_pre,
+                                                            const uint32_t* __restrict__ c_bm, int nbr, int W, int nJ, int* __restrict__ word_cnt,
+                                                            unsigned long long* __restrict__ flop_out, FilterArgs F) {
+  __shared__ KRec recs[4][64];
   const int lane = threadIdx.x & 63;
   const int64_t wv = ((int64_t)blockIdx.x * blockDim.x + threadIdx.x) >> 6;
-  unsigned long long flop = 0;
-  if (wv < (int64_t)nbr * nJ) {
-    const int i = (int)(wv / nJ), jb = (int)(wv % nJ);
-    const int j = jb * 64 + lane, w = j >> 5, bit = j & 31;
-    const uint32_t cw = w < W ? c_bm[(size_t)i * W + w] : 0u;
-    const bool present = (cw >> bit) & 1u;
-    if (__ballot(present)) {
-      const int a0 = a_row_p[i], a1 = a_row_p[i + 1];
-      const float reps = F.a_norms ? row_filter_eps(F, a1 - a0) : 0.0f;
-      int cnt = 0;
-      long long ksum = 0;
-      for (int ab = a0; ab < a1; ++ab) {
-        const int k = a_col_i[ab];
-        const uint32_t bw = w < W ? b_bm[(size_t)k * W + w] : 0u;
-        if ((bw >> bit) & 1u) {
-          if (F.a_norms) {
-            const int bidx = b_row_p[k] + b_pre[(size_t)k * W + w] + __popc(bw & ((1u << bit) - 1u));
-            if (F.a_norms[ab] * F.b_norms[bidx] < reps) continue;
-          }
-          ++cnt;
-          ksum += ks[k];
-        }
-      }
-      if (present) {
-        const int cb = c_row_p[i] + c_pre[(size_t)i * W + w] + __popc(cw & ((1u << bit) - 1u));
-        const int m = rs[i], n = cs[j];
-        prod_cnt[cb] = cnt;
-        blk_nze[cb] = m * n;
-        flop = 2ull * (unsigned long long)m * n * (unsigned long long)ksum;
-      }
-    }
-  }
-  __shared__ unsigned long long red[4];
+  if (wv >= (int64_t)nbr * nJ) return;
+  const int i = (int)(wv / nJ), jb = (int)(wv % nJ);
+  int a0;
+  unsigned long long cmask;
+  const GridWalk g = grid_walk_setup(lane, i, jb, W, a_row_p, c_bm, F, recs[threadIdx.x >> 6], &a0, &cmask);
+  int cnt = 0;
+  long long ksum = 0;
+  if (cmask)
+    for (int base = a0; base < g.a1; base += 64) {
+      unsigned long long hits = grid_walk_chunk(g, base, a_col_i, a_blk_p, ks, b_row_p, b_bm, b_pre, F);
+      if (F.a_norms) hits = grid_filter_hits(g, hits, F);
+      cnt += __popcll(hits);
+      for (; hits; hits &= hits - 1) ksum += g.rec[__ffsll((long long)hits) - 1].ks;
+    }
+  int c0 = lane < 32 ? cnt : 0, c1 = cnt - c0;
+  c0 = wave_sum(c0), c1 = wave_sum(c1);
+  if (lane == 0) {
+    word_cnt[(size_t)i * W + g.w0] = c0;
+    if (g.has1) word_cnt[(size_t)i * W + g.w0 + 1] = c1;
+  }
+  unsigned long long flop = g.present ? 2ull * (unsigned long long)rs[i] * (unsigned long long)cs[jb * 64 + lane] * (unsigned long long)ksum : 0ull;
   flop = wave_sum(flop);
-  if ((threadIdx.x & 63) == 0) red[threadIdx.x >> 6] = flop;
-  __syncthreads();
-  if (threadIdx.x == 0) {
-    const unsigned long long t = red[0] + red[1] + red[2] + red[3];
-    if (t) atomicAdd(flop_out, t);
-  }
+  if (lane == 0 && flop) atomicAdd(flop_out, flop);
 }
 
 __global__ void __launch_bounds__(256)
-fill_products_grid(const int* __restrict__ a_row_p, const int* __restrict__ a_col_i, const int64_t* __restrict__ a_blk_p,
+list_products_grid(const int* __restrict__ a_row_p, const int* __restrict__ a_col_i, const int64_t* __restrict__ a_blk_p,
                    const int* __restrict__ b_row_p, const int64_t* __restrict__ b_blk_p, const int* __restrict__ cin_row_p,
                    const int64_t* __restrict__ cin_blk_p, const int* __restrict__ rs, const int* __restrict__ ks,
                    const int* __restrict__ cs, const uint32_t* __restrict__ b_bm, const int* __restrict__ b_pre,
                    const uint32_t* __restrict__ cin_bm, const int* __restrict__ cin_pre, const uint32_t* __restrict__ c_bm,
-                   const int* __restrict__ c_pre, const int* __restrict__ c_row_p, const int64_t* __restrict__ prod_start,
-                   const int64_t* __restrict__ c_blk_p_ws, int nbr, int nbc, int W, int nJ, int* __restrict__ c_col_i,
+                   const int* __restrict__ c_pre, const int* __restrict__ c_row_p, const int64_t* __restrict__ word_pstart,
+                   const int64_t* __restrict__ word_cstart, int nbr, int W, int nJ, int stage_cap, int* __restrict__ c_col_i,
                    int64_t* __restrict__ c_blk_p, Desc* __restrict__ descs, Entry* __restrict__ entries, FilterArgs F) {
+  extern __shared__ __attribute__((aligned(16))) uint32_t list_lds[];
   const int lane = threadIdx.x & 63;
   const int64_t wv = ((int64_t)blockIdx.x * blockDim.x + threadIdx.x) >> 6;
   if (wv >= (int64_t)nbr * nJ) return;
   const int i = (int)(wv / nJ), jb = (int)(wv % nJ);
-  const int j = jb * 64 + lane, w = j >> 5, bit = j & 31;
-  const uint32_t cw = w < W ? c_bm[(size_t)i * W + w] : 0u;
-  const bool present = (cw >> bit) & 1u;
-  if (!__ballot(present)) return;
-  const uint32_t below = (1u << bit) - 1u;
-  const int cb = present ? c_row_p[i] + c_pre[(size_t)i * W + w] + __popc(cw & below) : 0;
-  const int64_t p0 = present ? prod_start[cb] : 0;
-  const int a0 = a_row_p[i], a1 = a_row_p[i + 1];
-  const float reps = F.a_norms ? row_filter_eps(F, a1 - a0) : 0.0f;
+  uint32_t* my_lds = list_lds + (size_t)(threadIdx.x >> 6) * (64 * (sizeof(KRec) / 4) + 3 * (size_t)stage_cap);
+  Entry* stage = reinterpret_cast<Entry*>(my_lds + 64 * (sizeof(KRec) / 4));
+  int a0;
+  unsigned long long cmask;
+  const GridWalk g = grid_walk_setup(lane, i, jb, W, a_row_p, c_bm, F, reinterpret_cast<KRec*>(my_lds), &a0, &cmask);
+  if (!cmask) return;
+  const bool single = g.a1 - a0 <= 64;
   int cnt = 0;
-  for (int base = a0; base < a1; base += 64) {
-    const int top = min(base + 64, a1);
-    unsigned long long hits = 0ull;
-    for (int ab = base; ab < top; ++ab) {
-      const int k = a_col_i[ab];
-      const uint32_t bw = w < W ? b_bm[(size_t)k * W + w] : 0u;
-      if (present && ((bw >> bit) & 1u)) hits |= 1ull << (ab - base);
+  unsigned long long hits0 = 0ull;
+  for (int base = a0; base < g.a1; base += 64) {
+    unsigned long long hits = grid_walk_chunk(g, base, a_col_i, a_blk_p, ks, b_row_p, b_bm, b_pre, F);
+    if (F.a_norms) hits = grid_filter_hits(g, hits, F);
+    cnt += __popcll(hits);
+    hits0 = hits;
+  }
+  const int j = jb * 64 + lane;
+  const int n = g.present ? cs[j] : 0, m = rs[i];
+  int inc = cnt;
+  int64_t einc = (int64_t)m * n;
+#pragma unroll
+  for (int off = 1; off < 64; off <<= 1) {
+    const int t = __shfl_up(inc, off, 64);
+    const int64_t te = __shfl_up(einc, off, 64);
+    if (lane >= off) inc += t, einc += te;
+  }
+  const int total = __shfl(inc, 63, 64);
+  const size_t t0 = (size_t)i * W + g.w0;
+  const int64_t wave_p0 = word_pstart[t0];
+  const int first = inc - cnt;
+  const bool staged = stage_cap > 0 && total <= stage_cap;
+  Entry* out = entries + wave_p0 + first;
+  Entry* lds_out = stage + first;
+  int at = 0;
+  for (int base = a0; base < g.a1; base += 64) {
+    unsigned long long hits = hits0;
+    if (!single) {
+      hits = grid_walk_chunk(g, base, a_col_i, a_blk_p, ks, b_row_p, b_bm, b_pre, F);
+      if (F.a_norms) hits = grid_filter_hits(g, hits, F);
     }
     while (hits) {
-      const int ab = base + __ffsll((long long)hits) - 1;
-      hits &= hits - 1;
-      const int k = a_col_i[ab];
-      const uint32_t bw = b_bm[(size_t)k * W + w];
-      const int bidx = b_row_p[k] + b_pre[(size_t)k * W + w] + __popc(bw & below);
-      if (F.a_norms && F.a_norms[ab] * F.b_norms[bidx] < reps) continue;
-      entries[p0 + cnt] = Entry::make(a_blk_p[ab], b_blk_p[bidx], ks[k]);
-      ++cnt;
-    }
-  }
-  if (present) {
+      KRec r[4];
+      int64_t b_off[4];
+      bool live[4];
+#pragma unroll
+      for (int u = 0; u < 4; ++u) {
+        live[u] = hits != 0ull;
+        const int l = live[u] ? __ffsll((long long)hits) - 1 : 0;
+        hits &= hits - 1;
+        r[u] = g.rec[l];
+      }
+#pragma unroll
+      for (int u = 0; u < 4; ++u) b_off[u] = live[u] ? b_blk_p[grid_b_index(g, r[u])] : 0;
+#pragma unroll
+      for (int u = 0; u < 4; ++u)
+        if (live[u]) {
+          const Entry e = Entry::make(r[u].a_off, b_off[u], r[u].ks);
+          if (staged)
+            lds_out[at] = e;
+          else
+            out[at] = e;
+          ++at;
+        }
+    }
+  }
+  if (staged) {
+    DBCSR_AMD_LDS_ORDER();
+    __builtin_amdgcn_wave_barrier();
+    const uint32_t* src = reinterpret_cast<const uint32_t*>(stage);
+    uint32_t* dst = reinterpret_cast<uint32_t*>(entries + wave_p0);
+    for (int q = lane; q < 3 * total; q += 64) dst[q] = src[q];
+  }
+  if (g.present) {
+    const int cb = c_row_p[i] + c_pre[t0] + __popcll(cmask & ((1ull << lane) - 1ull));
     Desc d;
-    d.c_off = c_blk_p_ws[cb];
+    d.c_off = word_cstart[t0] + einc - (int64_t)m * n;
     d.cin_off = -1;
     if (cin_bm) {
-      const uint32_t cinw = cin_bm[(size_t)i * W + w];
-      if ((cinw >> bit) & 1u) d.cin_off = cin_blk_p[cin_row_p[i] + cin_pre[(size_t)i * W + w] + __popc(cinw & below)];
-    }
-    d.prod_start = p0;
+      const size_t t = t0 + (lane >> 5);
+      const uint32_t cinw = cin_bm[t];
+      if ((cinw >> (lane & 31)) & 1u) d.cin_off = cin_blk_p[cin_row_p[i] + cin_pre[t] + __popc(cinw & g.below)];
+    }
+    d.prod_start = wave_p0 + first;
     d.prod_cnt = cnt;
-    d.m = (int16_t)rs[i];
-    d.n = (int16_t)cs[j];
+    d.m = (int16_t)m;
+    d.n = (int16_t)n;
     descs[cb] = d;
     c_col_i[cb] = j;
     c_blk_p[cb] = d.c_off;
@@ -503,8 +664,8 @@
 emit_index(const int* __restrict__ cin_row_p, const int64_t* __restrict__ cin_blk_p, const int* __restrict__ rs,
            const int* __restrict__ cs, const uint32_t* __restrict__ cin_bm, const int* __restrict__ cin_pre,
            const uint32_t* __restrict__ c_bm, const int* __restrict__ c_pre, const int* __restrict__ c_row_p,
-           const int64_t* __restrict__ c_blk_p_ws, int nbr, int W, int* __restrict__ c_col_i, int64_t* __restrict__ c_blk_p,
-           Desc* __restrict__ descs) {
+           const int64_t* __restrict__ c_blk_p_ws, const int64_t* __restrict__ word_cstart, int nbr, int W, int* __restrict__ c_col_i,
+           int64_t* __restrict__ c_blk_p, Desc* __restrict__ descs) {
   const int64_t t = (int64_t)blockIdx.x * blockDim.x + threadIdx.x;
   if (t >= (int64_t)nbr * W) return;
   const int i = (int)(t / W), w = (int)(t % W);
@@ -512,13 +673,15 @@
   if (!v) return;
   int cb = c_row_p[i] + c_pre[t];
   const uint32_t cinw = cin_bm ? cin_bm[t] : 0u;
+  int64_t off = word_cstart ? word_cstart[t] : 0;
   while (v) {
     const int bit = __ffs(v) - 1;
     v &= v - 1;
     const uint32_t below = (1u << bit) - 1u;
     const int j = 32 * w + bit;
     Desc d;
-    d.c_off = c_blk_p_ws[cb];
+    d.c_off = word_cstart ? off : c_blk_p_ws[cb];
+    off += (int64_t)rs[i] * cs[j];
     d.cin_off = -1;
     if ((cinw >> bit) & 1u) d.cin_off = cin_blk_p[cin_row_p[i] + cin_pre[t] + __popc(cinw & below)];
     d.prod_start = 0;
diff --git a/dbcsr_amd/csrc/mm_workspace.h b/dbcsr_amd/csrc/mm_workspace.h
--- a/dbcsr_amd/csrc/mm_workspace.h
+++ b/dbcsr_amd/csrc/mm_workspace.h
@@ -59,7 +59,8 @@
   return woff + inc - v;
 }
 
-__global__ void __launch_bounds__(kScanThreads) scan_reduce(const int* __restrict__ in, int64_t n, int64_t* __restrict__ partial) {
+template <typename TI>
+__global__ void __launch_bounds__(kScanThreads) scan_reduce(const TI* __restrict__ in, int64_t n, int64_t* __restrict__ partial) {
   const int64_t base = (int64_t)blockIdx.x * kScanChunk;
   int64_t s = 0;
   for (int it = 0; it < kScanItems; ++it) {
@@ -84,12 +85,12 @@
   if (threadIdx.x == 0 && total_out) *total_out = carry;
 }
 
-template <typename TO>
-__global__ void __launch_bounds__(kScanThreads) scan_apply(const int* __restrict__ in, int64_t n, const int64_t* __restrict__ partial,
+template <typename TO, typename TI>
+__global__ void __launch_bounds__(kScanThreads) scan_apply(const TI* __restrict__ in, int64_t n, const int64_t* __restrict__ partial,
                                                             TO* __restrict__ out, int write_total_at_n) {
   const int64_t base = (int64_t)blockIdx.x * kScanChunk;
   const int64_t first = base + (int64_t)threadIdx.x * kScanItems;
-  int v[kScanItems];
+  TI v[kScanItems];
   int64_t s = 0;
 #pragma unroll
   for (int it = 0; it < kScanItems; ++it) {
```
